# SebastianHafner/greedy_multimodal_learning

Measured on AMD Instinct MI355X. Metric: multi-view images/sec + step ms, ModelNet40 2-view MVCNN+MMTM @1/2/4/8 GPU, higher is better.
Workload: dtype bf16; 1 GPU; C2: 2-view MVCNN(ResNet-18 x2)+MMTM x3, guided gating (training_guided.gin eps 0.01, window 5, unlocked; decided on bf16-trunk gradients: d_BDR within ~6.5e-3 of eps may decide unlike fp32, INTEGRATION.md section 3); params=23773008, global_batch=64, per_gpu_batch=64, image=224, parallelism=dp1, hipgraph=True, device_gate=True

## Files before the change

greedy_multimodal_learning_amd/_lib.py:

```python
import ctypes
import os

import torch

_PKG = os.path.dirname(os.path.abspath(__file__))
LIB_PATH = os.path.join(_PKG, "libgreedymml_hip.so")

GM_F32, GM_BF16 = 0, 1
GM_NCHW, GM_NHWC = 0, 1
ABI_VERSION = 5

c_int, c_float, c_void_p, c_size_t = ctypes.c_int, ctypes.c_float, ctypes.c_void_p, ctypes.c_size_t
c_float_p = ctypes.c_void_p


class SpatialReduce(ctypes.Structure):
    _fields_ = [("x", c_void_p), ("dy", c_void_p), ("C", c_int), ("HW", c_int),
                ("out", c_void_p), ("ld_out", c_int), ("e", c_void_p), ("ld_e", c_int),
                ("scale", c_float)]


class ChannelScale(ctypes.Structure):
    _fields_ = [("x", c_void_p), ("y", c_void_p), ("C", c_int), ("HW", c_int),
                ("s", c_void_p), ("ld_s", c_int), ("a", c_void_p), ("ld_a", c_int),
# ... 104 lines not shown
    "gm_wprep_tiles": (c_int, [c_int, c_int, c_int]),
    "gm_conv_weight_prep_multi_bf16": (c_int, [c_void_p, c_int, c_int, c_void_p]),
})


class ConvDescHW(ctypes.Structure):
    _fields_ = [("N", c_int), ("H", c_int), ("W", c_int), ("C", c_int), ("K", c_int), ("R", c_int), ("S", c_int),
                ("stride_h", c_int), ("stride_w", c_int), ("pad_h", c_int), ("pad_w", c_int)]


EXPORTS.update({
    "gm_conv2d_fwd_hw_bf16": (c_int, [c_void_p, c_void_p, c_void_p, c_void_p, c_void_p]),
    "gm_conv2d_splitk_ws_bytes": (c_size_t, [c_void_p, c_int]),
    "gm_conv2d_fwd_ex_bf16": (c_int, [c_void_p, c_void_p, c_void_p, c_void_p, c_void_p, c_size_t, c_void_p]),
    "gm_conv2d_dgrad_ex_bf16": (c_int, [c_void_p, c_void_p, c_void_p, c_void_p, c_void_p, c_size_t, c_void_p]),
    "gm_conv2d_dgrad_add_bf16": (c_int, [c_void_p, c_void_p, c_void_p, c_void_p, c_void_p, c_void_p, c_size_t,
                                         c_void_p]),
    "gm_conv2d_wgrad_hw_scratch": (c_size_t, [c_void_p]),
    "gm_conv2d_fwd_grouped_bf16": (c_int, [c_void_p, c_int, c_void_p, c_void_p, ctypes.c_longlong, c_void_p,
                                           c_void_p, c_size_t, c_void_p]),
    "gm_conv2d_dgrad_grouped_bf16": (c_int, [c_void_p, c_int, c_void_p, c_void_p, ctypes.c_longlong, c_void_p,
                                             c_void_p, c_void_p, c_size_t, c_void_p]),
    "gm_conv2d_dgrad_grouped_masked_bf16": (c_int, [c_void_p, c_int, c_void_p, c_void_p, ctypes.c_longlong,
                                                    c_void_p, c_void_p, c_void_p, c_void_p, c_size_t, c_void_p]),
    "gm_conv2d_splitk_ws_bytes_grouped": (c_size_t, [c_void_p, c_int, c_int]),
    "gm_conv2d_wgrad_grouped_scratch": (c_size_t, [c_void_p, c_int]),
    "gm_conv2d_wgrad_grouped_bf16": (c_int, [c_void_p, c_int, c_void_p, c_void_p, c_void_p, ctypes.c_longlong,
                                             c_int, c_int, c_void_p, c_size_t, c_void_p]),
    "gm_conv2d_wgrad_hw_bf16": (c_int, [c_void_p, c_void_p, c_void_p, c_void_p, c_int, c_int, c_void_p,
                                        c_size_t, c_void_p]),
    "gm_stem_dw_crop": (c_int, [c_void_p, c_int, c_int, c_int, c_int, c_int, c_int, c_void_p, c_int, c_void_p]),
    "gm_conv2d_wgrad_stem_bn_ok": (c_int, [c_void_p, c_int]),
    "gm_conv2d_wgrad_stem_bn_grouped_bf16": (c_int, [c_void_p, c_int, c_void_p, c_void_p, c_void_p,
                                                     ctypes.c_longlong, c_int, c_void_p, c_size_t, c_void_p]),
})


class StemBnSrc(ctypes.Structure):
    _fields_ = [("y", c_void_p), ("dy_pool", c_void_p), ("idx", c_void_p), ("fcoef", c_void_p),
                ("fcoef_gs", ctypes.c_longlong), ("bcoef", c_void_p), ("bcoef_gs", ctypes.c_longlong)]


class WPrep(ctypes.Structure):
    _fields_ = [("w", c_void_p), ("wb", c_void_p), ("wt", c_void_p), ("K", c_int), ("RS", c_int),
                ("C", c_int), ("Cp", c_int), ("tile_start", c_int), ("pad", c_int)]


class GateState(ctypes.Structure):
    _fields_ = [("curation_mode", c_int), ("caring", c_int), ("curation_step", c_int), ("unlock", c_int),
                ("window", c_int), ("n_curated", c_int), ("pad0", c_int), ("pad1", c_int),
                ("eps", ctypes.c_double), ("M", ctypes.c_double * 4), ("d_bdr", ctypes.c_double)]


GATE_MAX_BRANCHES = 16


class GateStateN(ctypes.Structure):
    _fields_ = [("curation_mode", c_int), ("caring", c_int), ("curation_step", c_int), ("unlock", c_int),
                ("window", c_int), ("n_curated", c_int), ("nb", c_int), ("pad0", c_int),
                ("eps", ctypes.c_double), ("M_bypass", ctypes.c_double * GATE_MAX_BRANCHES),
                ("M_main", ctypes.c_double * GATE_MAX_BRANCHES), ("bdr", ctypes.c_double * GATE_MAX_BRANCHES),
                ("d_bdr", ctypes.c_double)]


class StemPack(ctypes.Structure):
    _fields_ = [("x", c_void_p), ("dtype", c_int), ("N", c_int), ("C0", c_int), ("H", c_int), ("W", c_int),
                ("pad", c_int), ("sn", ctypes.c_longlong), ("sc", ctypes.c_longlong), ("sh", ctypes.c_longlong),
                ("sw", ctypes.c_longlong), ("Hp", c_int), ("Wp", c_int), ("xp", c_void_p), ("w", c_void_p),
                ("K", c_int), ("R", c_int), ("S", c_int), ("wp", c_void_p), ("wk", ctypes.c_longlong),
                ("wc", ctypes.c_longlong), ("wr", ctypes.c_longlong), ("ws", ctypes.c_longlong)]


EXPORTS.update({
    "gm_gate_strong_step": (c_int, [c_void_p, c_void_p, c_void_p]),
    "gm_gate_strong_step_n": (c_int, [c_void_p, c_void_p, c_void_p]),
    "gm_mmtm_channel_scale_gated_n": (c_int, [c_void_p, c_int, c_int, c_int, c_int, c_void_p, c_void_p, c_void_p,
                                              c_void_p]),
    "gm_mmtm_spatial_reduce_gated_n": (c_int, [c_void_p, c_int, c_int, c_int, c_int, c_void_p, c_void_p, c_void_p,
                                               ctypes.c_size_t, c_void_p]),
    "gm_mmtm_select_scale": (c_int, [c_void_p, c_int, c_void_p, c_int, c_void_p, c_void_p, c_int, c_int, c_int,
                                     c_void_p, c_void_p, c_void_p, c_void_p, c_void_p]),
    "gm_mmtm_mask_rows": (c_int, [c_void_p, ctypes.c_longlong, c_void_p, c_void_p]),
    "gm_mmtm_mask_rows2": (c_int, [c_void_p, ctypes.c_longlong, c_void_p, ctypes.c_longlong, c_void_p, c_void_p]),
    "gm_mmtm_channel_scale_gated": (c_int, [c_void_p, c_int, c_int, c_int, c_int, c_void_p, c_void_p, c_void_p,
                                            c_void_p]),
    "gm_mmtm_spatial_reduce_gated": (c_int, [c_void_p, c_int, c_int, c_int, c_int, c_void_p, c_void_p, c_size_t,
                                             c_void_p]),
    "gm_stem_pack_bf16": (c_int, [c_void_p, c_void_p]),
    "gm_stem_pack_grouped_bf16": (c_int, [c_void_p, c_int, c_void_p]),
    "gm_xent_fwd": (c_int, [c_void_p, c_int, c_int, c_int, c_void_p, c_void_p, c_void_p, c_void_p]),
    "gm_xent_bwd": (c_int, [c_void_p, c_void_p, c_int, c_int, c_int, c_void_p, c_void_p, c_void_p, c_void_p]),
})


class BnFwd(ctypes.Structure):
    _fields_ = [("M", ctypes.c_longlong), ("C", c_int), ("relu", c_int), ("x", c_void_p),
                ("residual", c_void_p), ("y", c_void_p), ("gamma", c_void_p), ("beta", c_void_p),
                ("running_mean", c_void_p), ("running_var", c_void_p), ("momentum", c_float),
                ("eps", c_float), ("save_mean", c_void_p), ("save_invstd", c_void_p),
                ("num_batches_tracked", c_void_p), ("coef_out", c_void_p), ("relu_mask", c_void_p)]


class BnBwd(ctypes.Structure):
    _fields_ = [("M", ctypes.c_longlong), ("C", c_int), ("relu", c_int), ("dy", c_void_p),
                ("y", c_void_p), ("x", c_void_p), ("gamma", c_void_p), ("save_mean", c_void_p),
                ("save_invstd", c_void_p), ("dx", c_void_p), ("dres", c_void_p), ("dgamma", c_void_p),
                ("dbeta", c_void_p), ("accumulate", c_int), ("pad", c_int), ("fwd_coef", c_void_p),
                ("relu_mask", c_void_p)]


EXPORTS.update({
    "gm_bn_scratch": (c_size_t, [ctypes.c_longlong, c_int]),
    "gm_bn_fwd_train_bf16": (c_int, [c_void_p, c_void_p, c_size_t, c_void_p]),
    "gm_bn_fwd_stats_bf16": (c_int, [c_void_p, c_void_p, c_size_t, c_void_p]),
    "gm_bn_scratch_grouped": (c_size_t, [ctypes.c_longlong, c_int, c_int]),
    "gm_bn_fwd_train_grouped_bf16": (c_int, [c_void_p, c_int, c_void_p, c_size_t, c_void_p]),
    "gm_bn_bwd_grouped_bf16": (c_int, [c_void_p, c_int, c_void_p, c_size_t, c_void_p]),
    "gm_bn_fwd_stats_grouped_bf16": (c_int, [c_void_p, c_int, c_void_p, c_size_t, c_void_p]),
    "gm_bn_fwd_infer_bf16": (c_int, [c_void_p, c_void_p, c_size_t, c_void_p]),
    "gm_bn_bwd_bf16": (c_int, [c_void_p, c_void_p, c_size_t, c_void_p]),
})


class PoolDesc(ctypes.Structure):
    _fields_ = [("N", c_int), ("H", c_int), ("W", c_int), ("C", c_int), ("k", c_int), ("stride", c_int),
                ("pad", c_int)]


EXPORTS.update({
    "gm_maxpool2d_fwd_bf16": (c_int, [c_void_p, c_void_p, c_void_p, c_void_p, c_void_p]),
    "gm_bn_relu_maxpool2d_fwd_bf16": (c_int, [c_void_p, c_void_p, c_void_p, c_void_p, c_void_p, c_void_p]),
    "gm_bn_relu_maxpool2d_fwd_grouped_bf16": (c_int, [c_void_p, c_int, c_void_p, c_void_p, c_void_p, c_void_p,
                                                      c_void_p, c_void_p]),
    "gm_bn_relu_maxpool2d_bwd_grouped_bf16": (c_int, [c_void_p, c_int, c_void_p, c_void_p, c_void_p, c_void_p,
                                                      c_void_p, c_size_t, c_void_p]),
    "gm_bn_relu_maxpool2d_bwd_stats_grouped_bf16": (c_int, [c_void_p, c_int, c_void_p, c_void_p, c_void_p,
                                                            c_void_p, c_void_p, c_size_t, c_void_p, c_void_p,
                                                            c_void_p]),
    "gm_conv_stem_stats_rows": (c_int, [c_void_p, c_int]),
    "gm_conv2d_fwd_grouped_stats_bf16": (c_int, [c_void_p, c_int, c_void_p, c_void_p, ctypes.c_longlong, c_void_p,
                                                 c_void_p, c_int, c_void_p]),
    "gm_bn_fwd_stats_finalize_grouped": (c_int, [c_void_p, c_int, c_void_p, c_int, c_void_p]),
    "gm_conv2d_fwd_bn_stats_floats": (c_size_t, [c_void_p, c_int]),
    "gm_conv2d_fwd_grouped_bn_stats_bf16": (c_int, [c_void_p, c_int, c_void_p, c_void_p, ctypes.c_longlong, c_void_p,
                                                    c_void_p, c_size_t, c_void_p, c_void_p, c_size_t, c_void_p]),
    "gm_bn_fwd_apply_grouped_bf16": (c_int, [c_void_p, c_int, c_void_p, c_int, c_void_p]),
    "gm_conv2d_dgrad_bn_stats_floats": (c_size_t, [c_void_p, c_int]),
    "gm_conv2d_dgrad_grouped_bn_stats_bf16": (c_int, [c_void_p, c_int, c_void_p, c_void_p, ctypes.c_longlong,
                                                      c_void_p, c_void_p, c_void_p, c_void_p, c_void_p, c_size_t,
                                                      c_void_p, c_void_p, c_size_t, c_void_p]),
    "gm_bn_bwd_stats_coef_offset": (c_size_t, [c_int, c_int, c_int]),
    "gm_bn_bwd_stats_finalize_grouped": (c_int, [c_void_p, c_int, c_void_p, c_int, c_void_p]),
    "gm_bn_bwd_apply_grouped_bf16": (c_int, [c_void_p, c_int, c_void_p, c_int, c_void_p]),
    "gm_maxpool2d_bwd_bf16": (c_int, [c_void_p, c_void_p, c_void_p, c_void_p, c_void_p]),
})


class ConvF32(ctypes.Structure):
    _fields_ = [("mode", c_int), ("d", ConvDesc), ("x", c_void_p), ("w", c_void_p), ("dy", c_void_p),
                ("out", c_void_p), ("addend", c_void_p), ("accumulate", c_int), ("pad0", c_int)]


GM_CONV_FWD, GM_CONV_DGRAD, GM_CONV_WGRAD = 0, 1, 2

EXPORTS.update({
    "gm_conv2d_f32_scratch": (c_size_t, [c_void_p]),
    "gm_conv2d_f32": (c_int, [c_void_p, c_void_p, c_size_t, c_void_p]),
    "gm_conv2d_f32_split_scratch": (c_size_t, [c_void_p, c_int]),
    "gm_conv2d_f32_split": (c_int, [c_void_p, c_int, c_void_p, c_size_t, c_void_p]),
    "gm_conv2d_f32_affine": (c_int, [c_void_p, c_int, c_void_p, c_void_p, c_int, c_void_p, c_size_t, c_void_p]),
    "gm_bn_fwd_train_f32": (c_int, [c_void_p, c_void_p, c_size_t, c_void_p]),
    "gm_bn_fwd_infer_f32": (c_int, [c_void_p, c_void_p, c_size_t, c_void_p]),
    "gm_bn_bwd_f32": (c_int, [c_void_p, c_void_p, c_size_t, c_void_p]),
    "gm_maxpool2d_fwd_f32": (c_int, [c_void_p, c_void_p, c_void_p, c_void_p, c_void_p]),
    "gm_maxpool2d_bwd_f32": (c_int, [c_void_p, c_void_p, c_void_p, c_void_p, c_void_p]),
})

GM_FAULT_BN_SPIN, GM_FAULT_SPLITK_SPIN, GM_FAULT_CHAIN_SPIN = 1, 2, 4

EXPORTS.update({
    "gm_device_faults": (c_int, [ctypes.POINTER(ctypes.c_uint), c_int]),
    "gm_set_spin_limit": (c_int, [ctypes.c_uint]),
    "gm_bn_set_concurrency": (c_int, [c_int]),
    "gm_bn_set_fused_mode": (c_int, [c_int]),
    "gm_set_residency": (c_int, [c_int, c_int, c_int]),
    "gm_get_residency": (c_int, [ctypes.POINTER(c_int), ctypes.POINTER(c_int), ctypes.POINTER(c_int)]),
})


def set_residency(streams=None, sharers=None, reserved_cus=None):
    cur = get_residency()
    new = (cur[0] if streams is None else int(streams), cur[1] if sharers is None else int(sharers),
           cur[2] if reserved_cus is None else int(reserved_cus))
    check(load().gm_set_residency(*new), "gm_set_residency")
    return new


def get_residency():
    a, b, c = c_int(0), c_int(0), c_int(0)
    check(load().gm_get_residency(ctypes.byref(a), ctypes.byref(b), ctypes.byref(c)), "gm_get_residency")
    return a.value, b.value, c.value


_fault_reset_hooks = []


def on_fault_reset(fn):
    _fault_reset_hooks.append(fn)
    return fn


def device_faults(clear=False):
    v = ctypes.c_uint(0)
    check(load().gm_device_faults(ctypes.byref(v), int(clear)), "gm_device_faults")
    return v.value


def check_device_faults(clear=True):
    v = device_faults(clear)
    if v:
        for hook in _fault_reset_hooks:
            hook()
        what = [n for b, n in ((GM_FAULT_BN_SPIN, "fused BatchNorm coefficient hand-off"),
                               (GM_FAULT_SPLITK_SPIN, "split-K convolution turnstile"),
                               (GM_FAULT_CHAIN_SPIN, "chained GEMM hand-off")) if v & b]
        raise GreedyMMLError(f"device fault 0x{v:x}: {', '.join(what) or 'unknown'} timed out "
                             "(grid not co-resident?); the affected outputs are NaN")


class ViewsNorm(ctypes.Structure):
    _fields_ = [("x", c_void_p), ("flip", c_void_p), ("B", c_int), ("V", c_int), ("H", c_int), ("W", c_int),
                ("C", c_int), ("mean", c_float * 4), ("std", c_float * 4), ("out", c_void_p), ("dtype", c_int),
                ("layout", c_int)]


EXPORTS.update({
    "gm_views_normalize": (c_int, [c_void_p, c_void_p]),
})

EXPORTS.update({
    "gm_conv_set_halo": (c_int, [c_int]),
    "gm_conv_set_h9": (c_int, [c_int]),
    "gm_conv_set_wgrad_staging": (c_int, [c_int]),
    "gm_conv_set_splitk": (c_int, [c_int]),
    "gm_conv_set_wgrad_loop": (c_int, [c_int]),
    "gm_conv_set_1x1_gemm": (c_int, [c_int]),
    "gm_conv_set_rw": (c_int, [c_int]),
    "gm_conv_set_stem": (c_int, [c_int]),
    "gm_conv_set_wgrad_stem": (c_int, [c_int]),
})


class BnCoefEntry(ctypes.Structure):
    _fields_ = [("gamma", c_void_p), ("beta", c_void_p), ("running_mean", c_void_p), ("running_var", c_void_p),
                ("coef", c_void_p), ("C", c_int), ("eps", c_float)]


EXPORTS.update({
    "gm_bn_infer_coef": (c_int, [c_void_p, c_int, c_int, c_void_p]),
    "gm_conv2d_fwd_affine_ok": (c_int, [c_void_p, c_int]),
    "gm_conv2d_fwd_grouped_affine_bf16": (c_int, [c_void_p, c_int, c_void_p, c_void_p, ctypes.c_longlong, c_void_p,
                                                  c_void_p, ctypes.c_longlong, c_void_p, c_int, c_void_p, c_size_t,
                                                  c_void_p]),
    "gm_eval_metrics": (c_int, [c_void_p, c_int, c_int, c_int, c_void_p, c_void_p, c_void_p]),
})
```

greedy_multimodal_learning_amd/csrc/batchnorm.hip:

```cpp
#include <cstdlib>
#include <initializer_list>
#include <type_traits>

#include "gm_common.h"

namespace gm {
namespace {

constexpr int kT = 256;
constexpr int kMaxC = 2048;
constexpr size_t kHdr = 256;
constexpr int kMaxRC = 512;
constexpr int kRedF = 4096;

struct Plan {
    int SW, tpr_log, rpp;
    int nslice, nrc;
    long long rpb;
    size_t off_coef, off_p1, bytes;
};

inline int ilog2(int v) {
    int l = 0;
    while ((1 << l) < v) ++l;
// ... 98 lines not shown
    const float* gamma;
    const float* beta;
    float* rmean;
    float* rvar;
    float momentum, eps;
    float* save_mean;
    float* save_invstd;
    float* dgamma;
    float* dbeta;
    unsigned* counter;
    long long* nbt;
    float* coef;
    float* part;
    float* coef_out;
    const float* fcoef;
    unsigned* gen;
    const uint4* res;
    uint4* yout;
    uint4* dres_out;
    uint8_t* mask_out;
    const uint8_t* ymask;
    unsigned spin_limit;
    int redundant;
    unsigned long long scr_stride;
    unsigned hdr_words;
    BnGroup grp[kMaxBnG];
};

__device__ __forceinline__ ReduceArgs group_args(const ReduceArgs& a0) {
    ReduceArgs a = a0;
    const int g = blockIdx.z;
    const BnGroup& q = a0.grp[g];
    a.x = q.x; a.dy = q.dy; a.y = q.y;
    a.gamma = q.gamma; a.beta = q.beta; a.rmean = q.rmean; a.rvar = q.rvar;
    a.save_mean = q.save_mean; a.save_invstd = q.save_invstd;
    a.dgamma = q.dgamma; a.dbeta = q.dbeta; a.nbt = q.nbt;
    a.coef_out = q.coef_out; a.fcoef = q.fcoef;
    a.res = q.res; a.yout = q.yout; a.dres_out = q.dres_out;
    a.mask_out = q.mask_out; a.ymask = q.ymask;
    const unsigned long long off = (unsigned long long)g * a0.scr_stride;
    a.counter = a0.counter + g * a0.hdr_words;
    a.coef = reinterpret_cast<float*>(reinterpret_cast<char*>(a0.coef) + off);
    a.part = reinterpret_cast<float*>(reinterpret_cast<char*>(a0.part) + off);
    if (a0.gen) a.gen = a0.gen + g * a0.hdr_words;
    return a;
}

__device__ unsigned g_bn_fault = 0;

__device__ __forceinline__ bool wait_generation(const unsigned* gen, unsigned g0, unsigned limit, float* flag) {
    if (threadIdx.x == 0) {
        unsigned it = 0;
        bool ok = true;
        while (__hip_atomic_load(gen, __ATOMIC_RELAXED, __HIP_MEMORY_SCOPE_AGENT) == g0) {
            if (++it >= limit) {
                ok = false;
                break;
            }
            __builtin_amdgcn_s_sleep(2);
        }
        if (!ok) atomicOr(&g_bn_fault, GM_FAULT_BN_SPIN);
        *flag = ok ? 1.f : 0.f;
    }
    __syncthreads();
    return *flag != 0.f;
}

enum { FWD = 0, BWD = 1, BWD_RELU = 2, BWD_RELUX = 3 };

template <int MODE, typename E>
__device__ __forceinline__ void accum(const ReduceArgs& a, long long v, const float* mu, float* s1, float* s2,
                                      const float* fsc, const float* fsh) {
    float xf[8];
    V8<E>::ld(a.x, v, xf);
    if (MODE == FWD) {
#pragma unroll
        for (int j = 0; j < 8; ++j) {
            s1[j] += xf[j];
            s2[j] = fmaf(xf[j], xf[j], s2[j]);
        }
    } else {
        float d[8];
        V8<E>::ld(a.dy, v, d);
        if (MODE == BWD_RELU) {
            float yf[8];
            V8<E>::ld(a.y, v, yf);
#pragma unroll
            for (int j = 0; j < 8; ++j) d[j] = yf[j] > 0.f ? d[j] : 0.f;
        }
        if (MODE == BWD_RELUX) {
#pragma unroll
            for (int j = 0; j < 8; ++j) d[j] = fmaf(xf[j], fsc[j], fsh[j]) > 0.f ? d[j] : 0.f;
        }
#pragma unroll
        for (int j = 0; j < 8; ++j) {
            s1[j] += d[j];
            s2[j] = fmaf(d[j], xf[j] - mu[j], s2[j]);
        }
    }
}

template <int MODE>
__device__ __forceinline__ void accum_vals(uint4 ux, uint4 ud, uint4 uy, const float* mu, float* s1, float* s2,
                                          const float* fsc = nullptr, const float* fsh = nullptr) {
    float xf[8];
    unpack8(ux, xf);
    if (MODE == FWD) {
#pragma unroll
        for (int j = 0; j < 8; ++j) {
            s1[j] += xf[j];
            s2[j] = fmaf(xf[j], xf[j], s2[j]);
        }
    } else {
        float d[8];
        unpack8(ud, d);
        if (MODE == BWD_RELU) {
            float yf[8];
            unpack8(uy, yf);
#pragma unroll
            for (int j = 0; j < 8; ++j) d[j] = yf[j] > 0.f ? d[j] : 0.f;
        }
        if (MODE == BWD_RELUX) {
#pragma unroll
            for (int j = 0; j < 8; ++j) d[j] = fmaf(xf[j], fsc[j], fsh[j]) > 0.f ? d[j] : 0.f;
        }
#pragma unroll
        for (int j = 0; j < 8; ++j) {
            s1[j] += d[j];
            s2[j] = fmaf(d[j], xf[j] - mu[j], s2[j]);
        }
    }
}

struct FinOps {
    float g, b, rm, rv;
};

template <int MODE>
__device__ __forceinline__ FinOps fin_load(const ReduceArgs& a, int c) {
    FinOps f;
    f.g = a.gamma[c];
    if (MODE == FWD) {
        f.b = a.beta[c];
        f.rm = a.rmean ? a.rmean[c] : 0.f;
        f.rv = a.rmean ? a.rvar[c] : 0.f;
    } else {
        f.b = 0.f;
        f.rm = a.save_mean[c];
        f.rv = a.save_invstd[c];
    }
    return f;
}

template <int MODE, bool SC1 = false, bool CENTER = false>
__device__ __forceinline__ void finalize(const ReduceArgs& a, int c, double S1, double S2, double invM,
                                         const FinOps& f) {
    const int C = a.C;
    const double g = (double)f.g;
    if (MODE == FWD) {
        const double mean = S1 * invM;
        double var = S2 * invM - mean * mean;
        if (var < 0.0) var = 0.0;
        const double invstd = 1.0 / sqrt(var + (double)a.eps);
        const double sc = g * invstd;
        a.coef[c] = (float)sc;
        a.coef[C + c] = (float)((double)f.b - mean * sc);
        if (SC1) {
            st_sc1(&a.coef[c], a.coef[c]);
            st_sc1(&a.coef[C + c], a.coef[C + c]);
        }
        if (a.coef_out) {
            a.coef_out[c] = a.coef[c];
            a.coef_out[C + c] = a.coef[C + c];
        }
        a.save_mean[c] = (float)mean;
        a.save_invstd[c] = (float)invstd;
        if (a.rmean) {
            const double m = (double)a.momentum;
            const double unb = a.M > 1 ? var * (double)a.M / (double)(a.M - 1) : var;
            a.rmean[c] = (float)((1.0 - m) * (double)f.rm + m * mean);
            a.rvar[c] = (float)((1.0 - m) * (double)f.rv + m * unb);
        }
    } else {
        const double mean = (double)f.rm;
        const double is = (double)f.rv;
        const double ca = g * is;
        const double cb = -g * is * is * is * S2 * invM;
        a.coef[c] = (float)ca;
        a.coef[C + c] = (float)cb;
        if (CENTER) {
            a.coef[2 * C + c] = (float)(-ca * S1 * invM);
            a.coef[3 * C + c] = (float)mean;
        } else {
            a.coef[2 * C + c] = (float)(-ca * S1 * invM - cb * mean);
        }
        if (SC1) {
            st_sc1(&a.coef[c], a.coef[c]);
            st_sc1(&a.coef[C + c], a.coef[C + c]);
            st_sc1(&a.coef[2 * C + c], a.coef[2 * C + c]);
        }
        const float dg = (float)(S2 * is), db = (float)S1;
        if (a.accumulate) {
            a.dgamma[c] += dg;
            a.dbeta[c] += db;
        } else {
            a.dgamma[c] = dg;
            a.dbeta[c] = db;
        }
    }
}


__device__ __forceinline__ bool ticket(unsigned* ctr, unsigned n, float* flag) {
    asm volatile("s_waitcnt vmcnt(0)" ::: "memory");
    __syncthreads();
    if (threadIdx.x == 0) {
        const unsigned tk = __hip_atomic_fetch_add(ctr, 1u, __ATOMIC_RELAXED, __HIP_MEMORY_SCOPE_AGENT);
        const bool last = tk == n - 1;
        if (last) __hip_atomic_store(ctr, 0u, __ATOMIC_RELAXED, __HIP_MEMORY_SCOPE_AGENT);
        *flag = last ? 1.f : 0.f;
    }
    __syncthreads();
    return *flag != 0.f;
}

template <int MODE, bool SC1 = false>
__device__ __forceinline__ void combine_finalize(const ReduceArgs& a, int cs, float* red, const FinOps& fo);

template <int MODE, typename E>
__global__ __launch_bounds__(kT) void k_bn_reduce(ReduceArgs a0) {
    const ReduceArgs a = group_args(a0);
    __shared__ float red[kRedF + 4];
    const int t = threadIdx.x;
    const int C = a.C, SW = a.SW;
    const int rc = blockIdx.x, cs = blockIdx.y;
    const int tpr = 1 << a.tpr_log;
    const int cg = t & (tpr - 1);
    const int r0 = t >> a.tpr_log;
    const int rpp = kT >> a.tpr_log;
    const long long vpr = C >> 3;
    const int c0 = cs * SW + cg * 8;

    float fsc[8], fsh[8];
    if (MODE == BWD_RELUX) {
#pragma unroll
        for (int j = 0; j < 8; ++j) {
            fsc[j] = a.fcoef[c0 + j];
            fsh[j] = a.fcoef[C + c0 + j];
        }
    }
    float mu[8];
    if (MODE != FWD) {
#pragma unroll
        for (int j = 0; j < 8; ++j) mu[j] = a.save_mean[c0 + j];
    }
    float s1[8], s2[8];
#pragma unroll
    for (int j = 0; j < 8; ++j) s1[j] = s2[j] = 0.f;

    const long long rbeg = (long long)rc * a.rpb;
    long long rend = rbeg + a.rpb;
    if (rend > a.M) rend = a.M;
    long long r = rbeg + r0;
    const long long cv = c0 >> 3;
    const long long st = (long long)rpp * vpr;
    for (; r + 7 * rpp < rend; r += 8 * rpp) {
        const long long v = r * vpr + cv;
#pragma unroll
        for (int u = 0; u < 8; ++u) accum<MODE, E>(a, v + u * st, mu, s1, s2, fsc, fsh);
    }
    if (MODE == FWD && std::is_same<E, uint16_t>::value && r < rend) {
        const uint4* X = static_cast<const uint4*>(a.x);
        uint4 vx[8];
        const uint4 z = make_uint4(0u, 0u, 0u, 0u);
#pragma unroll
        for (int u = 0; u < 8; ++u) vx[u] = X[(r + u * rpp < rend ? r + u * rpp : r) * vpr + cv];
#pragma unroll
        for (int u = 0; u < 8; ++u) accum_vals<MODE>(r + u * rpp < rend ? vx[u] : z, z, z, mu, s1, s2);
    } else {
        for (; r < rend; r += rpp) accum<MODE, E>(a, r * vpr + cv, mu, s1, s2, fsc, fsh);
    }

    const int S2w = 2 * SW;
#pragma unroll
    for (int j = 0; j < 8; ++j) {
        red[r0 * S2w + (cg * 8 + j) * 2] = s1[j];
        red[r0 * S2w + (cg * 8 + j) * 2 + 1] = s2[j];
    }
    __syncthreads();
    float* p1 = a.part + ((size_t)cs * a.nrc + rc) * S2w;
    if (t < S2w) {
        float acc = 0.f;
        for (int i = 0; i < rpp; ++i) acc += red[i * S2w + t];
        st_sc1(&p1[t], acc);
    }
    FinOps fo{};
    if (t < SW) fo = fin_load<MODE>(a, cs * SW + t);
    if (!ticket(a.counter + cs, (unsigned)a.nrc, &red[kRedF])) return;
    combine_finalize<MODE>(a, cs, red, fo);
}

template <int MODE, bool SC1>
__device__ __forceinline__ void combine_finalize(const ReduceArgs& a, int cs, float* red, const FinOps& fo) {
    const int t = threadIdx.x;
    const int SW = a.SW, S2w = 2 * SW;
    if (MODE == FWD && a.nbt && cs == 0 && t == 0) *a.nbt += 1;
    const int L = S2w >> 2, G = kT / L;
    const int lv = t % L, g = t / L;
    const auto rq = rsrc_of(a.part + (size_t)cs * a.nrc * S2w);
    double d0 = 0.0, d1 = 0.0, d2 = 0.0, d3 = 0.0;
    for (int i0 = g; i0 < a.nrc; i0 += 8 * G) {
        float4 v[8];
#pragma unroll
        for (int u = 0; u < 8; ++u) {
            const int i = i0 + u * G;
            v[u] = i < a.nrc ? ld_sc1_f32x4(rq, (unsigned)(i * S2w + 4 * lv) * 4u) : make_float4(0.f, 0.f, 0.f, 0.f);
        }
#pragma unroll
        for (int u = 0; u < 8; ++u) {
            d0 += (double)v[u].x; d1 += (double)v[u].y; d2 += (double)v[u].z; d3 += (double)v[u].w;
        }
    }
    __syncthreads();
    double* rd = reinterpret_cast<double*>(red);
    rd[g * S2w + 4 * lv + 0] = d0;
    rd[g * S2w + 4 * lv + 1] = d1;
    rd[g * S2w + 4 * lv + 2] = d2;
    rd[g * S2w + 4 * lv + 3] = d3;
    __syncthreads();
    if (t < SW) {
        double S1 = 0.0, S2 = 0.0;
        for (int i = 0; i < G; ++i) {
            S1 += rd[i * S2w + 2 * t];
            S2 += rd[i * S2w + 2 * t + 1];
        }
        finalize<MODE, SC1>(a, cs * SW + t, S1, S2, 1.0 / (double)a.M, fo);
    }
}

struct StemPoolGeo {
    int Ng, H, W, P, Q;
    long long items;
    long long ipb;
    const uint2* idx;
    const uint4* gp;
    const uint4* xs;
};

typedef unsigned u32x4v_t __attribute__((ext_vector_type(4)));
__device__ __forceinline__ uint4 ld_nt16(const uint4* p) {
    const u32x4v_t v = __builtin_nontemporal_load(reinterpret_cast<const u32x4v_t*>(p));
    return make_uint4(v.x, v.y, v.z, v.w);
}
__device__ __forceinline__ void st_nt16(uint4* p, uint4 v) {
    const u32x4v_t w = {v.x, v.y, v.z, v.w};
    __builtin_nontemporal_store(w, reinterpret_cast<u32x4v_t*>(p));
}

template <bool APPLY>
__global__ __launch_bounds__(kT) void k_stem_pool_bn_bwd(ReduceArgs a0, StemPoolGeo pg) {
    const ReduceArgs a = group_args(a0);
    __shared__ float red[kRedF + 4];
// ... 24 lines not shown
    for (int j = 0; j < 8; ++j) s1[j] = s2[j] = 0.f;
    struct Item {
        uint2 iv[4];
        uint4 gq[4], xv[4];
        int n, k, l, cg;
        unsigned okw;
    };
    const unsigned QC8 = (unsigned)pg.Q * C8, WC8 = (unsigned)pg.W * C8;
    auto load = [&](long long i64, Item& it) {
        const unsigned i = (unsigned)i64;
        const unsigned ob = i / (unsigned)C8;
        it.cg = (int)(i - ob * (unsigned)C8);
        const unsigned r1 = ob / (unsigned)pg.Q;
        it.l = (int)(ob - r1 * (unsigned)pg.Q);
        const unsigned nn = r1 / (unsigned)pg.P;
        it.k = (int)(r1 - nn * (unsigned)pg.P);
        it.n = (int)nn;
        const int k = it.k, l = it.l;
        const unsigned o0 = i;
        it.okw = 0u;
#pragma unroll
        for (int u = 0; u < 4; ++u) {
            const int wr = u >> 1, wc = u & 1;
            const bool ok = k + wr < pg.P && l + wc < pg.Q;
            const unsigned o = ok ? o0 + (unsigned)wr * QC8 + (unsigned)wc * (unsigned)C8 : o0;
            it.iv[u] = IDX[o];
            it.gq[u] = GP[o];
            it.okw |= ok ? (1u << u) : 0u;
        }
        const unsigned x0 = ((nn * (unsigned)pg.H + 2u * (unsigned)k) * (unsigned)pg.W + 2u * (unsigned)l) * C8 + it.cg;
#pragma unroll
        for (int q = 0; q < 4; ++q) {
            const int dh = q >> 1, dw = q & 1;
            const bool in = 2 * k + dh < pg.H && 2 * l + dw < pg.W;
            it.xv[q] = ld_nt16(&X[in ? x0 + (unsigned)dh * WC8 + (unsigned)dw * (unsigned)C8 : x0]);
        }
    };
    auto compute = [&](const Item& it) {
        const int n = it.n, k = it.k, l = it.l, cg = it.cg;
        float gv[4][8];
#pragma unroll
        for (int u = 0; u < 4; ++u) unpack8(it.gq[u], gv[u]);
        uint2 ivm[4];
#pragma unroll
        for (int u = 0; u < 4; ++u) ivm[u] = ((it.okw >> u) & 1u) ? it.iv[u] : make_uint2(~0u, ~0u);
#pragma unroll
        for (int q = 0; q < 4; ++q) {
            const int dh = q >> 1, dw = q & 1;
            const int h = 2 * k + dh, w = 2 * l + dw;
            if (h >= pg.H || w >= pg.W) continue;
            float d[8];
#pragma unroll
            for (int j = 0; j < 8; ++j) d[j] = 0.f;
#pragma unroll
            for (int u = 0; u < 4; ++u) {
                const int wr = u >> 1, wc = u & 1;
                if (wr > dh || wc > dw) continue;
                const uint32_t pos = (uint32_t)((dh - 2 * wr + 1) * 3 + (dw - 2 * wc + 1));
#pragma unroll
                for (int j = 0; j < 8; ++j) {
                    const uint32_t b = ((j < 4 ? ivm[u].x : ivm[u].y) >> (8 * (j & 3))) & 0xffu;
                    if (b == pos) d[j] += gv[u][j];
                }
            }
            float xf[8];
            unpack8(it.xv[q], xf);
#pragma unroll
            for (int j = 0; j < 8; ++j) {
                const float dr = __uint_as_float((uint32_t)Elem<uint16_t>::f2bf(d[j]) << 16);
                d[j] = fmaf(xf[j], fsc[j], fsh[j]) > 0.f ? dr : 0.f;
            }
            if (APPLY) {
                float o[8];
#pragma unroll
                for (int j = 0; j < 8; ++j) o[j] = fmaf(ca[j], d[j], fmaf(cb[j], xf[j], cc[j]));
                st_nt16(&reinterpret_cast<uint4*>(a.yout)[(((long long)n * pg.H + h) * pg.W + w) * C8 + cg], pack8(o));
            } else {
#pragma unroll
                for (int j = 0; j < 8; ++j) {
                    s1[j] += d[j];
                    s2[j] = fmaf(d[j], xf[j] - mu[j], s2[j]);
                }
            }
        }
    };
    auto item = [&](long long i) {
        Item it;
        load(i, it);
        compute(it);
    };
    if (APPLY) {
        const long long stride = (long long)gridDim.x * kT;
        long long i = (long long)blockIdx.x * kT + t;
        for (; i + stride < pg.items; i += 2 * stride) {
            Item u, v;
            load(i, u);
            load(i + stride, v);
            compute(u);
            compute(v);
        }
        if (i < pg.items) item(i);
        return;
    }
    const int rc = blockIdx.x;
    const long long i0 = (long long)rc * pg.ipb;
    const long long i1 = i0 + pg.ipb < pg.items ? i0 + pg.ipb : pg.items;
    if (pg.xs) {
        const uint4* __restrict__ XS = pg.xs + goff;
        for (long long i = i0 + t; i < i1; i += 4 * kT) {
            uint4 gq[4], xq[4];
#pragma unroll
            for (int u = 0; u < 4; ++u) {
                const long long iu = i + u * kT < i1 ? i + u * kT : i;
                gq[u] = GP[iu];
                xq[u] = XS[iu];
            }
#pragma unroll
            for (int u = 0; u < 4; ++u) {
                if (i + u * kT >= i1) break;
                float gv[8], xf[8];
                unpack8(gq[u], gv);
                unpack8(xq[u], xf);
#pragma unroll
                for (int j = 0; j < 8; ++j) {
                    const float d = fmaf(xf[j], fsc[j], fsh[j]) > 0.f ? gv[j] : 0.f;
                    s1[j] += d;
                    s2[j] = fmaf(d, xf[j] - mu[j], s2[j]);
                }
            }
        }
    } else {
        for (long long i = i0 + t; i < i1; i += kT) item(i);
    }
    const int S2w = 2 * C, r0 = t / C8, rpp = kT / C8;
#pragma unroll
    for (int j = 0; j < 8; ++j) {
        red[r0 * S2w + (cg0 * 8 + j) * 2] = s1[j];
        red[r0 * S2w + (cg0 * 8 + j) * 2 + 1] = s2[j];
    }
    __syncthreads();
    float* p1 = a.part + (size_t)rc * S2w;
    if (t < S2w) {
        float acc = 0.f;
        for (int i = 0; i < rpp; ++i) acc += red[i * S2w + t];
        st_sc1(&p1[t], acc);
    }
    FinOps fo{};
    if (t < C) fo = fin_load<BWD_RELUX>(a, t);
    if (!ticket(a.counter, (unsigned)a.nrc, &red[kRedF])) return;
    combine_finalize<BWD_RELUX>(a, 0, red, fo);
}

constexpr int kFinT = 1024;
__global__ __launch_bounds__(kFinT) void k_bn_stats_finalize(ReduceArgs a0) {
    const ReduceArgs a = group_args(a0);
    __shared__ double rd[kFinT / 32][128];
    const int t = threadIdx.x, cs = blockIdx.y;
    const int lv = t & 31, rg = t >> 5;
    FinOps fo;
    {
        const int c = cs * 64 + (t & 63);
        const float* rm = a.rmean ? a.rmean : a.gamma;
        const float* rv = a.rmean ? a.rvar : a.gamma;
        fo.g = a.gamma[c];
        fo.b = a.beta[c];
        fo.rm = rm[c];
        fo.rv = rv[c];
    }
    const float4* rows = reinterpret_cast<const float4*>(a.part + (size_t)cs * a.nrc * 128);
    double d0 = 0.0, d1 = 0.0, d2 = 0.0, d3 = 0.0;
    for (int i0 = rg; i0 < a.nrc; i0 += 8 * 32) {
        float4 v[8];
#pragma unroll
        for (int u = 0; u < 8; ++u) v[u] = rows[(size_t)min(i0 + u * 32, a.nrc - 1) * 32 + lv];
#pragma unroll
        for (int u = 0; u < 8; ++u) {
            if (i0 + u * 32 >= a.nrc) v[u] = make_float4(0.f, 0.f, 0.f, 0.f);
            d0 += (double)v[u].x; d1 += (double)v[u].y; d2 += (double)v[u].z; d3 += (double)v[u].w;
        }
    }
    rd[rg][4 * lv] = d0; rd[rg][4 * lv + 1] = d1; rd[rg][4 * lv + 2] = d2; rd[rg][4 * lv + 3] = d3;
    __syncthreads();
    if (t < 64) {
        double S1 = 0.0, S2 = 0.0;
        for (int i = 0; i < kFinT / 32; ++i) {
            S1 += rd[i][2 * t];
            S2 += rd[i][2 * t + 1];
        }
        finalize<FWD>(a, cs * 64 + t, S1, S2, 1.0 / (double)a.M, fo);
        if (a.nbt && cs == 0 && t == 0) *a.nbt += 1;
    }
}

__global__ __launch_bounds__(kFinT) void k_bn_bwd_stats_finalize(ReduceArgs a0, float* coef0, long long cstride) {
    ReduceArgs a = group_args(a0);
    a.coef = coef0 + blockIdx.z * cstride;
    __shared__ double rd[kFinT / 32][128];
    const int t = threadIdx.x, cs = blockIdx.y;
    const int lv = t & 31, rg = t >> 5;
    const FinOps fo = fin_load<BWD>(a, cs * 64 + (t & 63));
    const float4* rows = reinterpret_cast<const float4*>(a.part + (size_t)cs * a.nrc * 128);
    double d0 = 0.0, d1 = 0.0, d2 = 0.0, d3 = 0.0;
    for (int i0 = rg; i0 < a.nrc; i0 += 8 * 32) {
        float4 v[8];
#pragma unroll
        for (int u = 0; u < 8; ++u) v[u] = rows[(size_t)min(i0 + u * 32, a.nrc - 1) * 32 + lv];
#pragma unroll
        for (int u = 0; u < 8; ++u) {
            if (i0 + u * 32 >= a.nrc) v[u] = make_float4(0.f, 0.f, 0.f, 0.f);
            d0 += (double)v[u].x; d1 += (double)v[u].y; d2 += (double)v[u].z; d3 += (double)v[u].w;
        }
    }
    rd[rg][4 * lv] = d0; rd[rg][4 * lv + 1] = d1; rd[rg][4 * lv + 2] = d2; rd[rg][4 * lv + 3] = d3;
    __syncthreads();
    if (t < 64) {
        double S1 = 0.0, S2 = 0.0;
        for (int i = 0; i < kFinT / 32; ++i) {
            S1 += rd[i][2 * t];
            S2 += rd[i][2 * t + 1];
        }
        finalize<BWD>(a, cs * 64 + t, S1, S2, 1.0 / (double)a.M, fo);
    }
}

__device__ __forceinline__ bool arrive(unsigned* ctr, unsigned n, float* flag) {
    asm volatile("s_waitcnt vmcnt(0)" ::: "memory");
    __syncthreads();
    if (threadIdx.x == 0) {
        const unsigned tk = __hip_atomic_fetch_add(ctr, 1u, __ATOMIC_RELAXED, __HIP_MEMORY_SCOPE_AGENT);
        *flag = tk == n - 1 ? 1.f : 0.f;
    }
    __syncthreads();
    return *flag != 0.f;
}

__device__ __forceinline__ bool wait_count(unsigned* ctr, unsigned n, unsigned limit, float* flag) {
    if (threadIdx.x == 0) {
        unsigned it = 0;
        bool ok = true;
        while (__hip_atomic_load(ctr, __ATOMIC_RELAXED, __HIP_MEMORY_SCOPE_AGENT) < n) {
            if (++it >= limit) {
                ok = false;
                break;
            }
            __builtin_amdgcn_s_sleep(1);
        }
        if (!ok) atomicOr(&g_bn_fault, GM_FAULT_BN_SPIN);
        *flag = ok ? 1.f : 0.f;
    }
    __syncthreads();
    return *flag != 0.f;
}

__device__ __forceinline__ void depart(unsigned* ctr, unsigned n) {
    if (threadIdx.x == 0) {
        const unsigned tk = __hip_atomic_fetch_add(ctr, 1u, __ATOMIC_RELAXED, __HIP_MEMORY_SCOPE_AGENT);
        if (tk == 2 * n - 1) __hip_atomic_store(ctr, 0u, __ATOMIC_RELAXED, __HIP_MEMORY_SCOPE_AGENT);
    }
}

template <int MODE>
__device__ __forceinline__ void combine_coefs(const ReduceArgs& a, int cs, float* red, const FinOps& fo, bool last,
                                              float* cf) {
    const int t = threadIdx.x;
    const int SW = a.SW, S2w = 2 * SW;
    const int L = S2w >> 2, G = kT / L;
    const int lv = t % L, g = t / L;
    const auto rq = rsrc_of(a.part + (size_t)cs * a.nrc * S2w);
    double d0 = 0.0, d1 = 0.0, d2 = 0.0, d3 = 0.0;
    for (int i0 = g; i0 < a.nrc; i0 += 8 * G) {
        float4 v[8];
#pragma unroll
        for (int u = 0; u < 8; ++u) {
            const int i = i0 + u * G;
            v[u] = i < a.nrc ? ld_sc1_f32x4(rq, (unsigned)(i * S2w + 4 * lv) * 4u) : make_float4(0.f, 0.f, 0.f, 0.f);
        }
#pragma unroll
        for (int u = 0; u < 8; ++u) {
            d0 += (double)v[u].x; d1 += (double)v[u].y; d2 += (double)v[u].z; d3 += (double)v[u].w;
        }
    }
    __syncthreads();
    double* rd = reinterpret_cast<double*>(red);
    rd[g * S2w + 4 * lv + 0] = d0;
    rd[g * S2w + 4 * lv + 1] = d1;
    rd[g * S2w + 4 * lv + 2] = d2;
    rd[g * S2w + 4 * lv + 3] = d3;
    __syncthreads();
    if (t < SW) {
        double S1 = 0.0, S2 = 0.0;
        for (int i = 0; i < G; ++i) {
            S1 += rd[i * S2w + 2 * t];
            S2 += rd[i * S2w + 2 * t + 1];
        }
        const double invM = 1.0 / (double)a.M;
        const int c = cs * SW + t;
        if (last) {
            if (MODE == FWD && a.nbt && cs == 0 && t == 0) *a.nbt += 1;
            finalize<MODE, false>(a, c, S1, S2, invM, fo);
        }
        const double gg = (double)fo.g;
        if (MODE == FWD) {
            const double mean = S1 * invM;
            double var = S2 * invM - mean * mean;
            if (var < 0.0) var = 0.0;
            const double invstd = 1.0 / sqrt(var + (double)a.eps);
            const double sc = gg * invstd;
            cf[t] = (float)sc;
            cf[SW + t] = (float)((double)fo.b - mean * sc);
        } else {
            const double mean = (double)fo.rm, is = (double)fo.rv;
            const double ca = gg * is, cb = -gg * is * is * is * S2 * invM;
            cf[t] = (float)ca;
            cf[SW + t] = (float)cb;
            cf[2 * SW + t] = (float)(-ca * S1 * invM - cb * mean);
        }
    }
    __syncthreads();
}

template <int MODE>
__global__ __launch_bounds__(kT) void k_bn_reduce_f64(ReduceArgs a0) {
    const ReduceArgs a = group_args(a0);
    __shared__ double red[kRedF];
    __shared__ float flag;
    const int t = threadIdx.x;
    const int C = a.C, SW = a.SW;
    const int rc = blockIdx.x, cs = blockIdx.y;
    const int tpr = 1 << a.tpr_log;
    const int cg = t & (tpr - 1);
    const int r0 = t >> a.tpr_log;
    const int rpp = kT >> a.tpr_log;
    const long long vpr = C >> 3;
    const int c0 = cs * SW + cg * 8;
    const float* X = static_cast<const float*>(a.x);
    const float* DY = static_cast<const float*>(a.dy);
    const float* Y = static_cast<const float*>(a.y);
    double fsc[8], fsh[8], mu[8], s1[8], s2[8];
#pragma unroll
    for (int j = 0; j < 8; ++j) {
        fsc[j] = MODE == BWD_RELUX ? (double)a.fcoef[c0 + j] : 0.0;
        fsh[j] = MODE == BWD_RELUX ? (double)a.fcoef[C + c0 + j] : 0.0;
        mu[j] = MODE != FWD ? (double)a.save_mean[c0 + j] : 0.0;
        s1[j] = s2[j] = 0.0;
    }
    const long long rbeg = (long long)rc * a.rpb;
    long long rend = rbeg + a.rpb;
    if (rend > a.M) rend = a.M;
    for (long long r = rbeg + r0; r < rend; r += rpp) {
        const long long e = r * C + c0;
        float xf[8], d[8];
        V8<float>::ld(X + e, 0, xf);
        if (MODE != FWD) V8<float>::ld(DY + e, 0, d);
        if (MODE == BWD_RELU) {
            float yf[8];
            V8<float>::ld(Y + e, 0, yf);
#pragma unroll
            for (int j = 0; j < 8; ++j) d[j] = yf[j] > 0.f ? d[j] : 0.f;
        }
#pragma unroll
        for (int j = 0; j < 8; ++j) {
            if (MODE == BWD_RELUX) d[j] = fmaf(xf[j], (float)fsc[j], (float)fsh[j]) > 0.f ? d[j] : 0.f;
            if (MODE == FWD) {
                s1[j] += (double)xf[j];
                s2[j] = fma((double)xf[j], (double)xf[j], s2[j]);
            } else {
                s1[j] += (double)d[j];
                s2[j] = fma((double)d[j], (double)xf[j] - mu[j], s2[j]);
            }
        }
    }
    const int S2w = 2 * SW;
#pragma unroll
    for (int j = 0; j < 8; ++j) {
// ... 217 lines not shown
            unsigned wm[US];
#pragma unroll
            for (int u = 0; u < US; ++u) {
                const long long i = r * vpr + cv + u * st;
                wx[u] = X[i];
                wd[u] = DY[i];
                if (MODE == BWD_RELU && YM) wm[u] = a.ymask[i];
                else if (MODE == BWD_RELU) wy[u] = Y[i];
            }
#pragma unroll
            for (int u = 0; u < US; ++u) {
                pin(wx[u]);
                pin(wd[u]);
                if (MODE == BWD_RELU && YM) pin(wm[u]);
                else if (MODE == BWD_RELU) pin(wy[u]);
            }
#pragma unroll
            for (int u = 0; u < US; ++u)
                accum_vals<MODE>(wx[u], wd[u], MODE == BWD_RELU ? (YM ? mask_vals(wm[u]) : wy[u]) : z, mu, s1, s2, fsc,
                                 fsh);
        }
        for (; r < rend; r += rpp) {
            const long long i = r * vpr + cv;
            accum_vals<MODE>(X[i], DY[i], MODE == BWD_RELU ? ldy(i) : z, mu, s1, s2, fsc, fsh);
        }
    }

    const int S2w = 2 * SW;
#pragma unroll
    for (int j = 0; j < 8; ++j) {
        red[r0 * S2w + (cg * 8 + j) * 2] = s1[j];
        red[r0 * S2w + (cg * 8 + j) * 2 + 1] = s2[j];
    }
    __syncthreads();
    float* p1 = a.part + ((size_t)cs * a.nrc + rc) * S2w;
    if (t < S2w) {
        float acc = 0.f;
        for (int i = 0; i < rpp; ++i) acc += red[i * S2w + t];
        st_sc1(&p1[t], acc);
    }
    FinOps fo{};
    if (t < SW) fo = fin_load<MODE>(a, cs * SW + t);
    bool fresh = true;
    float ca[8], cb[8], cc[8];
    if (a.redundant) {
        __shared__ float cf[3 * 64];
        const bool last = arrive(a.counter + cs, (unsigned)a.nrc, &red[kRedF]);
        fresh = wait_count(a.counter + cs, (unsigned)a.nrc, a.spin_limit, &red[kRedF + 1]);
        combine_coefs<MODE>(a, cs, red, fo, last, cf);
        depart(a.counter + cs, (unsigned)a.nrc);
#pragma unroll
        for (int j = 0; j < 8; ++j) {
            ca[j] = cf[cg * 8 + j];
            cb[j] = cf[SW + cg * 8 + j];
            cc[j] = cf[2 * SW + cg * 8 + j];
        }
    } else {
        if (ticket(a.counter + cs, (unsigned)a.nrc, &red[kRedF])) {
            combine_finalize<MODE, true>(a, cs, red, fo);
            asm volatile("s_waitcnt vmcnt(0)" ::: "memory");
            __syncthreads();
            if (t == 0) __hip_atomic_store(gen, g0 + 1u, __ATOMIC_RELAXED, __HIP_MEMORY_SCOPE_AGENT);
        } else {
            fresh = wait_generation(gen, g0, a.spin_limit, &red[kRedF + 1]);
        }
        const auto rq = rsrc_of(a.coef);
        auto ld8 = [&](int off, float* o) {
            const float4 p = ld_sc1_f32x4(rq, (unsigned)(off + c0) * 4u), q = ld_sc1_f32x4(rq, (unsigned)(off + c0 + 4) * 4u);
            o[0] = p.x; o[1] = p.y; o[2] = p.z; o[3] = p.w; o[4] = q.x; o[5] = q.y; o[6] = q.z; o[7] = q.w;
        };
        ld8(0, ca);
        ld8(C, cb);
        ld8(2 * C, cc);
    }
    if (!fresh) {
#pragma unroll
        for (int j = 0; j < 8; ++j) ca[j] = cb[j] = cc[j] = __builtin_nanf("");
    }
    auto out = [&](uint4 ux, uint4 ud, uint4 uy, long long i) {
        float d[8], xf[8];
        unpack8(ud, d);
        unpack8(ux, xf);
        if (MODE == BWD_RELU) {
            float yf[8];
            unpack8(uy, yf);
#pragma unroll
            for (int j = 0; j < 8; ++j) d[j] = yf[j] > 0.f ? d[j] : 0.f;
        }
        if (MODE == BWD_RELUX) {
#pragma unroll
            for (int j = 0; j < 8; ++j) d[j] = fmaf(xf[j], fsc[j], fsh[j]) > 0.f ? d[j] : 0.f;
        }
        if (DRES) a.dres_out[i] = pack8(d);
        float o[8];
#pragma unroll
        for (int j = 0; j < 8; ++j)
            o[j] = fmaf(ca[j], d[j], fmaf(cb[j], xf[j], cc[j]));
        a.yout[i] = pack8(o);
    };
    if (NR > 0) {
#pragma unroll
        for (int u = 0; u < NV; ++u) {
            const long long r = rbeg + r0 + (long long)u * rpp;
            if (r < rend) out(vx[u], vd[u], MODE == BWD_RELU ? vy[u < NY ? u : 0] : z, r * vpr + cv);
        }
    } else {
        long long r = rbeg + r0;
        const long long st = (long long)rpp * vpr;
        for (; r + (US - 1) * rpp < rend; r += US * rpp) {
            uint4 wx[US], wd[US], wy[US];
            unsigned wm[US];
#pragma unroll
            for (int u = 0; u < US; ++u) {
                const long long i = r * vpr + cv + u * st;
                wx[u] = X[i];
                wd[u] = DY[i];
                if (MODE == BWD_RELU && YM) wm[u] = a.ymask[i];
                else if (MODE == BWD_RELU) wy[u] = Y[i];
            }
#pragma unroll
            for (int u = 0; u < US; ++u) {
                pin(wx[u]);
                pin(wd[u]);
                if (MODE == BWD_RELU && YM) pin(wm[u]);
                else if (MODE == BWD_RELU) pin(wy[u]);
            }
#pragma unroll
            for (int u = 0; u < US; ++u)
                out(wx[u], wd[u], MODE == BWD_RELU ? (YM ? mask_vals(wm[u]) : wy[u]) : z, r * vpr + cv + u * st);
        }
        for (; r < rend; r += rpp) {
            const long long i = r * vpr + cv;
            out(X[i], DY[i], MODE == BWD_RELU ? ldy(i) : z, i);
        }
    }
}

struct ApplyArgs {
    long long nvec;
    int tpr_log;
    int relu;
    const void* x;
    const void* res;
    const void* dy;
    void* out;
    void* out2;
    const float* coef;
    int C;
    const float* fcoef;
    long long gvec;
    long long cgs;
    long long fcgs;
    uint8_t* mask_out;
};

__device__ __forceinline__ void load_coef(const float* p, int cg, float* c) {
    const float4 a = reinterpret_cast<const float4*>(p)[cg * 2];
    const float4 b = reinterpret_cast<const float4*>(p)[cg * 2 + 1];
    c[0] = a.x; c[1] = a.y; c[2] = a.z; c[3] = a.w; c[4] = b.x; c[5] = b.y; c[6] = b.z; c[7] = b.w;
}

template <bool RES, bool RELU, typename E>
__global__ __launch_bounds__(kT) void k_bn_apply(ApplyArgs a) {
    const long long stride = (long long)gridDim.x * kT;
    long long v = (long long)blockIdx.x * kT + threadIdx.x;
    const int cg = (int)(v & ((1 << a.tpr_log) - 1));
    const long long go = blockIdx.y * a.gvec;
    const float* coef = a.coef + blockIdx.y * a.cgs;
    float sc[8], sh[8];
    load_coef(coef, cg, sc);
    load_coef(coef + a.C, cg, sh);
    auto fin = [&](long long i, float* f, const float* r) {
#pragma unroll
        for (int j = 0; j < 8; ++j) {
            float z = fmaf(f[j], sc[j], sh[j]);
            if (RES) z += r[j];
            f[j] = RELU ? relu_nan(z) : z;
        }
        V8<E>::st(a.out, i, f);
        if (RES && RELU && std::is_same<E, uint16_t>::value && a.mask_out) a.mask_out[i] = (uint8_t)mask_byte(pack8(f));
    };
    auto one = [&](long long i) {
        i += go;
        float f[8];
        V8<E>::ld(a.x, i, f);
        float r[8];
        if (RES) V8<E>::ld(a.res, i, r);
        fin(i, f, r);
    };
    if constexpr (std::is_same<E, uint16_t>::value) {
        typedef unsigned u32x4 __attribute__((ext_vector_type(4)));
        constexpr int U = 4;
        const u32x4* XX = static_cast<const u32x4*>(a.x) + go;
        const u32x4* RR = static_cast<const u32x4*>(a.res) + go;
        for (; v + (U - 1) * stride < a.nvec; v += U * stride) {
            u32x4 rx[U], rr[U];
#pragma unroll
            for (int u = 0; u < U; ++u) {
                rx[u] = XX[v + u * stride];
                if (RES) rr[u] = RR[v + u * stride];
            }
#pragma unroll
            for (int u = 0; u < U; ++u) {
                asm volatile("" : "+v"(rx[u]));
                if (RES) asm volatile("" : "+v"(rr[u]));
            }
#pragma unroll
            for (int u = 0; u < U; ++u) {
                float f[8], r[8];
                unpack8(make_uint4(rx[u].x, rx[u].y, rx[u].z, rx[u].w), f);
                if (RES) unpack8(make_uint4(rr[u].x, rr[u].y, rr[u].z, rr[u].w), r);
                fin(go + v + u * stride, f, r);
            }
        }
        for (; v < a.nvec; v += stride) one(v);
        return;
    }
    for (; v + stride < a.nvec; v += 2 * stride) {
        one(v);
        one(v + stride);
    }
    if (v < a.nvec) one(v);
}

template <bool RELU, bool DRES, bool MASKX, typename E>
__global__ __launch_bounds__(kT) void k_bn_apply_bwd(ApplyArgs a) {
    constexpr bool CENTER = std::is_same<E, float>::value;
    const long long stride = (long long)gridDim.x * kT;
    long long v = (long long)blockIdx.x * kT + threadIdx.x;
    const int cg = (int)(v & ((1 << a.tpr_log) - 1));
    const long long go = blockIdx.y * a.gvec;
    const float* coef = a.coef + blockIdx.y * a.cgs;
    float ca[8], cb[8], cc[8], fs[8], fh[8], mu[8];
    load_coef(coef, cg, ca);
    load_coef(coef + a.C, cg, cb);
    load_coef(coef + 2 * a.C, cg, cc);
    if (CENTER) load_coef(coef + 3 * a.C, cg, mu);
    if (MASKX) {
        load_coef(a.fcoef + blockIdx.y * a.fcgs, cg, fs);
        load_coef(a.fcoef + blockIdx.y * a.fcgs + a.C, cg, fh);
    }
    constexpr bool YR = RELU && !MASKX;
    auto ld = [&](long long i, float* d, float* xf, float* yf) {
        V8<E>::ld(a.dy, go + i, d);
        V8<E>::ld(a.x, go + i, xf);
        if (YR) V8<E>::ld(a.res, go + i, yf);
    };
    auto out = [&](long long i, float* d, const float* xf, const float* yf) {
        if (RELU && MASKX) {
#pragma unroll
            for (int j = 0; j < 8; ++j) d[j] = fmaf(xf[j], fs[j], fh[j]) > 0.f ? d[j] : 0.f;
        } else if (RELU) {
#pragma unroll
            for (int j = 0; j < 8; ++j) d[j] = yf[j] > 0.f ? d[j] : 0.f;
        }
        if (DRES) V8<E>::st(a.out2, go + i, d);
        float o[8];
#pragma unroll
        for (int j = 0; j < 8; ++j)
            o[j] = CENTER ? fmaf(ca[j], d[j], fmaf(cb[j], xf[j] - mu[j], cc[j])) : fmaf(ca[j], d[j], fmaf(cb[j], xf[j], cc[j]));
        V8<E>::st(a.out, go + i, o);
    };
    constexpr int U = 4;
    if constexpr (std::is_same<E, uint16_t>::value) {
        typedef unsigned u32x4 __attribute__((ext_vector_type(4)));
        const u32x4* DY = static_cast<const u32x4*>(a.dy) + go;
        const u32x4* XX = static_cast<const u32x4*>(a.x) + go;
        const u32x4* YY = static_cast<const u32x4*>(a.res) + go;
        auto u4 = [](u32x4 w) { return make_uint4(w.x, w.y, w.z, w.w); };
        for (; v + (U - 1) * stride < a.nvec; v += U * stride) {
            u32x4 rd[U], rx[U], ry[U];
#pragma unroll
            for (int u = 0; u < U; ++u) {
                rd[u] = DY[v + u * stride];
                rx[u] = XX[v + u * stride];
                if (YR) ry[u] = YY[v + u * stride];
            }
#pragma unroll
            for (int u = 0; u < U; ++u) {
                asm volatile("" : "+v"(rd[u]), "+v"(rx[u]));
                if (YR) asm volatile("" : "+v"(ry[u]));
            }
#pragma unroll
            for (int u = 0; u < U; ++u) {
                float d[8], xf[8], yf[8];
                unpack8(u4(rd[u]), d);
                unpack8(u4(rx[u]), xf);
                if (YR) unpack8(u4(ry[u]), yf);
                out(v + u * stride, d, xf, yf);
            }
        }
    } else {
        for (; v + (U - 1) * stride < a.nvec; v += U * stride) {
            float d[U][8], xf[U][8], yf[U][YR ? 8 : 1];
#pragma unroll
            for (int u = 0; u < U; ++u) ld(v + u * stride, d[u], xf[u], yf[u]);
#pragma unroll
            for (int u = 0; u < U; ++u) out(v + u * stride, d[u], xf[u], yf[u]);
        }
    }
    for (; v < a.nvec; v += stride) {
        float d[8], xf[8], yf[YR ? 8 : 1];
        ld(v, d, xf, yf);
        out(v, d, xf, yf);
    }
}

__global__ void k_bn_infer_coef(int C, const float* gamma, const float* beta, const float* rm, const float* rv,
                                float eps, float* coef) {
    const int c = blockIdx.x * blockDim.x + threadIdx.x;
    if (c >= C) return;
    const double is = 1.0 / sqrt((double)rv[c] + (double)eps);
    const double sc = (double)gamma[c] * is;
    coef[c] = (float)sc;
    coef[C + c] = (float)((double)beta[c] - (double)rm[c] * sc);
}

__global__ void k_bn_infer_coef_table(const gm_bn_coef_entry* tab) {
    const gm_bn_coef_entry e = tab[blockIdx.y];
    const int c = blockIdx.x * blockDim.x + threadIdx.x;
    const int C = e.C;
    if (c >= C) return;
    const double is = 1.0 / sqrt((double)e.running_var[c] + (double)e.eps);
    const double sc = (double)e.gamma[c] * is;
    e.coef[c] = (float)sc;
// ... 397 lines not shown
    ReduceArgs a{};
    fill_fwd(a, ps, G, grouped, pl, static_cast<char*>(scratch));
    hipLaunchKernelGGL((k_bn_reduce<FWD, uint16_t>), dim3(pl.nrc, pl.nslice, G), dim3(kT), 0, as_stream(stream), a);
    return check_launch("k_bn_reduce<fwd>");
}

}

namespace gm {
unsigned bn_faults_read(bool clear) {
    unsigned v = 0;
    if (hipMemcpyFromSymbol(&v, HIP_SYMBOL(g_bn_fault), sizeof(v), 0, hipMemcpyDeviceToHost) != hipSuccess) return ~0u;
    if (clear && v) {
        const unsigned z = 0;
        (void)hipMemcpyToSymbol(HIP_SYMBOL(g_bn_fault), &z, sizeof(z), 0, hipMemcpyHostToDevice);
    }
    return v;
}
}

extern "C" int gm_bn_set_concurrency(int n) {
    GM_REQUIRE(n >= 1 && n <= 1024, "gm_bn_set_concurrency: n must be in [1, 1024] (got %d)", n);
    gm::g_concurrency = n;
    return GM_OK;
}

extern "C" int gm_bn_set_fused_mode(int mode) {
    GM_REQUIRE(mode >= 0 && mode <= 2, "gm_bn_set_fused_mode: mode must be 0, 1 or 2 (got %d)", mode);
    gm::g_fused_env = mode;
    return GM_OK;
}

extern "C" int gm_bn_fwd_stats_bf16(const gm_bn_fwd* p, void* scratch, size_t bytes, void* stream) {
    return bn_fwd_stats(p, 1, false, scratch, bytes, stream, "gm_bn_fwd_stats_bf16");
}

extern "C" size_t gm_bn_scratch_grouped(long long M, int C, int G) {
    if (M <= 0 || C < 8 || C > kMaxC || G < 1 || G > kMaxBnG) return 0;
    return grouped_bytes(M, C, G);
}

extern "C" int gm_bn_fwd_train_grouped_bf16(const gm_bn_fwd* ps, int G, void* scratch, size_t bytes, void* stream) {
    return bn_fwd_train<uint16_t>(ps, G, true, scratch, bytes, stream, "gm_bn_fwd_train_grouped_bf16");
}
extern "C" int gm_bn_bwd_grouped_bf16(const gm_bn_bwd* ps, int G, void* scratch, size_t bytes, void* stream) {
    return bn_bwd<uint16_t>(ps, G, true, scratch, bytes, stream, "gm_bn_bwd_grouped_bf16");
}
extern "C" int gm_bn_fwd_stats_grouped_bf16(const gm_bn_fwd* ps, int G, void* scratch, size_t bytes, void* stream) {
    return bn_fwd_stats(ps, G, true, scratch, bytes, stream, "gm_bn_fwd_stats_grouped_bf16");
}

extern "C" int gm_bn_fwd_train_bf16(const gm_bn_fwd* p, void* scratch, size_t bytes, void* stream) {
    return bn_fwd_train<uint16_t>(p, 1, false, scratch, bytes, stream, "gm_bn_fwd_train_bf16");
}
extern "C" int gm_bn_fwd_infer_bf16(const gm_bn_fwd* p, void* scratch, size_t bytes, void* stream) {
    return bn_fwd_infer<uint16_t>(p, scratch, bytes, stream, "gm_bn_fwd_infer_bf16");
}
extern "C" int gm_bn_bwd_bf16(const gm_bn_bwd* p, void* scratch, size_t bytes, void* stream) {
    return bn_bwd<uint16_t>(p, 1, false, scratch, bytes, stream, "gm_bn_bwd_bf16");
}
extern "C" int gm_bn_fwd_train_f32(const gm_bn_fwd* p, void* scratch, size_t bytes, void* stream) {
    return bn_fwd_train<float>(p, 1, false, scratch, bytes, stream, "gm_bn_fwd_train_f32");
}
extern "C" int gm_bn_infer_coef(const gm_bn_coef_entry* table, int n, int max_c, void* stream) {
    const char* fn = "gm_bn_infer_coef";
    GM_REQUIRE(table, "%s: null table", fn);
    GM_REQUIRE(n >= 1 && n <= 65535, "%s: n must be 1..65535 (got %d)", fn, n);
    GM_REQUIRE(max_c >= 1, "%s: max_c must be >= 1 (got %d)", fn, max_c);
    hipLaunchKernelGGL(k_bn_infer_coef_table, dim3((max_c + 255) / 256, n), dim3(256), 0, as_stream(stream), table);
    return check_launch("k_bn_infer_coef_table");
}

extern "C" int gm_bn_fwd_infer_f32(const gm_bn_fwd* p, void* scratch, size_t bytes, void* stream) {
    return bn_fwd_infer<float>(p, scratch, bytes, stream, "gm_bn_fwd_infer_f32");
}
extern "C" int gm_bn_bwd_f32(const gm_bn_bwd* p, void* scratch, size_t bytes, void* stream) {
    return bn_bwd<float>(p, 1, false, scratch, bytes, stream, "gm_bn_bwd_f32");
}

static int stem_pool_bwd(const gm_pool_desc* d, int G, const void* dy_pool, const void* idx, const void* xsel,
                         const gm_bn_bwd* ps, void* scratch, size_t bytes, bool apply, const float** bcoef,
                         long long* bcoef_gs, void* stream, const char* fn) {
    GM_REQUIRE(d && dy_pool && idx && ps && G >= 1 && G <= kMaxBnG, "%s: bad arguments", fn);
    GM_REQUIRE(d->k == 3 && d->stride == 2 && d->pad == 1 && d->C == 64 && d->N >= 1 && d->H >= 2 && d->W >= 2,
               "%s: the stem's pool only (k 3, stride 2, pad 1, C 64)", fn);
    const int P = (d->H + 2 - 3) / 2 + 1, Q = (d->W + 2 - 3) / 2 + 1;
    GM_REQUIRE((d->H + 1) / 2 == P && (d->W + 1) / 2 == Q, "%s: pool geometry", fn);
    for (int g = 0; g < G; ++g) {
        const gm_bn_bwd& p = ps[g];
        GM_REQUIRE(p.M == (long long)d->N * d->H * d->W && p.C == d->C && p.relu && p.fwd_coef && !p.y && !p.dres &&
                       p.x && (p.dx || !apply) && p.gamma && p.save_mean && p.save_invstd && p.dgamma && p.dbeta &&
                       p.accumulate == ps[0].accumulate,
                   "%s: group %d: BN backward must be M = N*H*W, C, relu with fwd_coef, no y / dres", fn, g);
    }
    int rc;
    if ((rc = check_scratch(ps[0].M, ps[0].C, G, true, scratch, bytes, fn))) return rc;
    const Plan pl = make_plan(ps[0].M, ps[0].C);
    ReduceArgs a{};
    a.M = ps[0].M; a.C = ps[0].C; a.relu = 1; a.SW = ps[0].C; a.tpr_log = 3;
    a.accumulate = ps[0].accumulate;
    set_scratch(a, pl, static_cast<char*>(scratch), true);
    for (int g = 0; g < G; ++g) {
        BnGroup& q = a.grp[g];
        q.x = ps[g].x;
        q.gamma = ps[g].gamma;
        q.save_mean = const_cast<float*>(ps[g].save_mean);
        q.save_invstd = const_cast<float*>(ps[g].save_invstd);
        q.dgamma = ps[g].dgamma; q.dbeta = ps[g].dbeta;
        q.fcoef = ps[g].fwd_coef;
        q.yout = static_cast<uint4*>(ps[g].dx);
    }
    StemPoolGeo pg;
    pg.Ng = d->N; pg.H = d->H; pg.W = d->W; pg.P = P; pg.Q = Q;
    pg.items = (long long)d->N * P * Q * (d->C / 8);
    GM_REQUIRE((long long)d->N * d->H * d->W * (d->C / 8) < (1ll << 31), "%s: a group's map exceeds 2^31 vectors", fn);
    int nrc = pl.nrc < kMaxRC ? pl.nrc : kMaxRC;
    pg.ipb = (pg.items + nrc - 1) / nrc;
    pg.ipb = (pg.ipb + kT - 1) / kT * kT;
    nrc = (int)((pg.items + pg.ipb - 1) / pg.ipb);
    a.nrc = nrc;
    pg.idx = static_cast<const uint2*>(idx);
    pg.gp = static_cast<const uint4*>(dy_pool);
    pg.xs = static_cast<const uint4*>(xsel);
    hipStream_t st = as_stream(stream);
    hipLaunchKernelGGL((k_stem_pool_bn_bwd<false>), dim3(nrc, 1, G), dim3(kT), 0, st, a, pg);
    if ((rc = check_launch("k_stem_pool_bn_bwd<reduce>"))) return rc;
    if (!apply) {
        *bcoef = a.coef;
        *bcoef_gs = (long long)(a.scr_stride / sizeof(float));
        return GM_OK;
    }
    long long grid = (pg.items + kT - 1) / kT;
    if (grid > 4096) grid = 4096;
    hipLaunchKernelGGL((k_stem_pool_bn_bwd<true>), dim3((unsigned)grid, 1, G), dim3(kT), 0, st, a, pg);
    return check_launch("k_stem_pool_bn_bwd<apply>");
}

extern "C" int gm_bn_relu_maxpool2d_bwd_grouped_bf16(const gm_pool_desc* d, int G, const void* dy_pool,
                                                     const void* idx, const void* xsel, const gm_bn_bwd* ps,
                                                     void* scratch, size_t bytes, void* stream) {
    return stem_pool_bwd(d, G, dy_pool, idx, xsel, ps, scratch, bytes, true, nullptr, nullptr, stream,
                         "gm_bn_relu_maxpool2d_bwd_grouped_bf16");
}

extern "C" int gm_bn_relu_maxpool2d_bwd_stats_grouped_bf16(const gm_pool_desc* d, int G, const void* dy_pool,
                                                           const void* idx, const void* xsel, const gm_bn_bwd* ps,
                                                           void* scratch, size_t bytes, const float** bcoef,
                                                           long long* bcoef_gs, void* stream) {
    const char* fn = "gm_bn_relu_maxpool2d_bwd_stats_grouped_bf16";
    GM_REQUIRE(bcoef && bcoef_gs, "%s: null coefficient outputs", fn);
    return stem_pool_bwd(d, G, dy_pool, idx, xsel, ps, scratch, bytes, false, bcoef, bcoef_gs, stream, fn);
}

extern "C" int gm_bn_fwd_stats_finalize_grouped(const gm_bn_fwd* ps, int G, float* stats, int rows, void* stream) {
    const char* fn = "gm_bn_fwd_stats_finalize_grouped";
    int rc = check_groups_fwd(ps, G, fn);
    if (rc) return rc;
    const int C = ps[0].C;
    GM_REQUIRE(stats && rows >= 1 && C >= 64 && C % 64 == 0 && ps[0].M >= 1, "%s: C a multiple of 64, rows >= 1",
               fn);
    ReduceArgs a{};
    a.M = ps[0].M; a.C = C; a.SW = 64; a.tpr_log = 3; a.nrc = rows;
    a.momentum = ps[0].momentum; a.eps = ps[0].eps;
    a.part = stats;
    a.coef = stats + (size_t)rows * 2 * C;
    a.scr_stride = (unsigned long long)(rows + 1) * 2 * C * sizeof(float);
    a.hdr_words = 0;
    for (int g = 0; g < G; ++g) {
        BnGroup& q = a.grp[g];
        q.x = ps[g].x;
        q.gamma = ps[g].gamma; q.beta = ps[g].beta;
        q.rmean = ps[g].running_mean; q.rvar = ps[g].running_var;
        q.save_mean = ps[g].save_mean; q.save_invstd = ps[g].save_invstd;
        q.nbt = ps[g].num_batches_tracked;
        q.coef_out = ps[g].coef_out;
    }
    hipLaunchKernelGGL(k_bn_stats_finalize, dim3(1, C / 64, G), dim3(kFinT), 0, as_stream(stream), a);
    return check_launch("k_bn_stats_finalize");
}

extern "C" int gm_bn_fwd_apply_grouped_bf16(const gm_bn_fwd* ps, int G, const float* stats, int rows, void* stream) {
    const char* fn = "gm_bn_fwd_apply_grouped_bf16";
    int rc = check_groups_fwd(ps, G, fn);
    if (rc) return rc;
    const gm_bn_fwd* p = ps;
    const int C = p->C;
    GM_REQUIRE(stats && rows >= 1 && C >= 64 && C % 64 == 0 && p->y, "%s: C a multiple of 64, rows >= 1, y", fn);
    const long long gs = p->M * C;
    bool strided = true;
    for (int g = 1; g < G; ++g) {
        const uint16_t* x0 = static_cast<const uint16_t*>(p->x);
        strided = strided && ps[g].x == x0 + g * gs &&
                  ps[g].y == static_cast<uint16_t*>(p->y) + g * gs &&
                  (!p->residual || ps[g].residual == static_cast<const uint16_t*>(p->residual) + g * gs) &&
                  (!p->relu_mask || ps[g].relu_mask == static_cast<uint8_t*>(p->relu_mask) + g * gs / 8);
    }
    const long long cgs = (long long)(rows + 1) * 2 * C;
    hipStream_t st = as_stream(stream);
    const int ng = strided ? 1 : G;
    for (int gi = 0; gi < ng; ++gi) {
        ApplyArgs b{};
        b.nvec = p->M * (C / 8); b.tpr_log = ilog2(C / 8); b.C = C; b.relu = p->relu;
        b.x = ps[gi].x; b.res = ps[gi].residual; b.out = ps[gi].y;
        b.mask_out = static_cast<uint8_t*>(ps[gi].relu_mask);
        b.coef = stats + gi * cgs + (size_t)rows * 2 * C;
        b.gvec = strided ? gs / 8 : 0;
        b.cgs = strided ? cgs : 0;
        const dim3 g(apply_grid(b.nvec, C), strided ? G : 1);
        if (p->residual) {
            if (p->relu) hipLaunchKernelGGL((k_bn_apply<true, true, uint16_t>), g, dim3(kT), 0, st, b);
            else hipLaunchKernelGGL((k_bn_apply<true, false, uint16_t>), g, dim3(kT), 0, st, b);
        } else {
            if (p->relu) hipLaunchKernelGGL((k_bn_apply<false, true, uint16_t>), g, dim3(kT), 0, st, b);
            else hipLaunchKernelGGL((k_bn_apply<false, false, uint16_t>), g, dim3(kT), 0, st, b);
        }
        if ((rc = check_launch("k_bn_apply"))) return rc;
    }
    return GM_OK;
}

extern "C" size_t gm_bn_bwd_stats_coef_offset(int C, int G, int rows) {
    return (size_t)G * 2 * C * (size_t)(rows + 1);
}

static int check_bwd_from_stats(const gm_bn_bwd* ps, int G, const float* stats, int rows, const char* fn) {
    int rc = check_groups_bwd(ps, G, fn);
    if (rc) return rc;
    const int C = ps[0].C;
    GM_REQUIRE(stats && rows >= 1 && C >= 64 && C % 64 == 0 && ps[0].M >= 1, "%s: C a multiple of 64, rows >= 1",
               fn);
    GM_REQUIRE(!ps[0].dres && (!ps[0].relu || ps[0].fwd_coef),
               "%s: relu needs fwd_coef (mask from x); no residual gradient", fn);
    return GM_OK;
}

extern "C" int gm_bn_bwd_stats_finalize_grouped(const gm_bn_bwd* ps, int G, float* stats, int rows, void* stream) {
    const char* fn = "gm_bn_bwd_stats_finalize_grouped";
    int rc = check_bwd_from_stats(ps, G, stats, rows, fn);
    if (rc) return rc;
    const int C = ps[0].C;
    ReduceArgs a{};
    a.M = ps[0].M; a.C = C; a.SW = 64; a.tpr_log = 3; a.nrc = rows;
    a.accumulate = ps[0].accumulate;
    a.part = stats;
    a.coef = stats;
    a.scr_stride = (unsigned long long)(rows + 1) * 2 * C * sizeof(float);
    a.hdr_words = 0;
    for (int g = 0; g < G; ++g) {
        BnGroup& q = a.grp[g];
        q.x = ps[g].x; q.dy = ps[g].dy;
        q.gamma = ps[g].gamma;
        q.save_mean = const_cast<float*>(ps[g].save_mean);
        q.save_invstd = const_cast<float*>(ps[g].save_invstd);
        q.dgamma = ps[g].dgamma; q.dbeta = ps[g].dbeta;
    }
    float* coef0 = stats + gm_bn_bwd_stats_coef_offset(C, G, rows);
    hipLaunchKernelGGL(k_bn_bwd_stats_finalize, dim3(1, C / 64, G), dim3(kFinT), 0, as_stream(stream), a, coef0,
                       (long long)4 * C);
    return check_launch("k_bn_bwd_stats_finalize");
}

extern "C" int gm_bn_bwd_apply_grouped_bf16(const gm_bn_bwd* ps, int G, const float* stats, int rows, void* stream) {
    const char* fn = "gm_bn_bwd_apply_grouped_bf16";
    int rc = check_bwd_from_stats(ps, G, stats, rows, fn);
    if (rc) return rc;
    const gm_bn_bwd* p = ps;
    const int C = p->C;
    GM_REQUIRE(p->dx && p->dy && p->x, "%s: null argument (dx, dy, x)", fn);
    const long long gs = p->M * C;
    bool strided = true;
    for (int g = 1; g < G; ++g)
        strided = strided && ps[g].x == static_cast<const uint16_t*>(p->x) + g * gs &&
                  ps[g].dy == static_cast<const uint16_t*>(p->dy) + g * gs &&
                  ps[g].dx == static_cast<uint16_t*>(p->dx) + g * gs &&
                  (!p->relu || ps[g].fwd_coef == p->fwd_coef + (size_t)g * 2 * C);
    const float* coef0 = stats + gm_bn_bwd_stats_coef_offset(C, G, rows);
    hipStream_t st = as_stream(stream);
    const int ng = strided ? 1 : G;
    for (int gi = 0; gi < ng; ++gi) {
        ApplyArgs b{};
        b.nvec = p->M * (C / 8); b.tpr_log = ilog2(C / 8); b.C = C; b.relu = p->relu;
        b.x = ps[gi].x; b.dy = ps[gi].dy; b.out = ps[gi].dx;
        b.coef = coef0 + (size_t)gi * 4 * C;
        b.fcoef = ps[gi].fwd_coef;
        b.gvec = strided ? gs / 8 : 0;
        b.cgs = strided ? 4 * C : 0;
        b.fcgs = strided ? 2 * C : 0;
        const dim3 g(apply_grid(b.nvec, C), strided ? G : 1);
        if (p->relu) hipLaunchKernelGGL((k_bn_apply_bwd<true, false, true, uint16_t>), g, dim3(kT), 0, st, b);
        else hipLaunchKernelGGL((k_bn_apply_bwd<false, false, false, uint16_t>), g, dim3(kT), 0, st, b);
        if ((rc = check_launch("k_bn_apply_bwd"))) return rc;
    }
    return GM_OK;
}
```

greedy_multimodal_learning_amd/vtrunk.py:

```python
import contextlib
import ctypes
import os

import torch

from .streams import zeroed_scratch
from . import _lib as L
from .bn import MASK_FROM_X
from .conv import CL, _cpad, _desc, _desc_hw, _like_param, _prepped, _splitk_ws, _stem_geom, stem_pack, \
    stem_pack_grouped
from .gradsink import GradJoin, MaskedAddend, sink_done, sink_pending, sink_target

BF = torch.bfloat16
ENABLED = os.environ.get("GM_VTRUNK", "1") != "0"


FUSED_STEM_BWD = True
STEM_XSEL = True
FUSED_STEM_WGRAD = True
FUSED_STEM_STATS = True
EPI_BN_STATS = True
BN_RELU_MASK = True
DS_DZ_LINK = True
IDT_MASKED_ADDEND = True
EPI_BN_BWD_STATS = True
_GM_E_UNSUP = -3


def _nhwc(t):
    return t if t.is_contiguous(memory_format=CL) else t.contiguous(memory_format=CL)


def _stride(ts, elem_bytes):
    if len(ts) < 2:
        return 0
    d = ts[1].data_ptr() - ts[0].data_ptr()
    if d == 0 or d % elem_bytes:
        return None
    for a, b in zip(ts[1:], ts[2:]):
        if b.data_ptr() - a.data_ptr() != d:
            return None
    return d // elem_bytes


def _splitk_g(device, d, G, dgrad):
    need = L.load().gm_conv2d_splitk_ws_bytes_grouped(ctypes.byref(d), G, int(dgrad))
    if need == 0:
        return 0, 0
    buf = zeroed_scratch(_splitk_ws, device, need, lambda old: (need + (1 << 20) - 1) >> 20 << 20)
    return buf.data_ptr(), buf.numel()


_bn_scratch = {}


def _bn_scratch_g(device, M, C, G):
    need = L.load().gm_bn_scratch_grouped(M, C, G)
    return zeroed_scratch(_bn_scratch, device, need,
                          lambda old: max(need, 1 << 20) if old is None else max(need, 2 * old.numel()))


@L.on_fault_reset
def _reset_bn_scratch():
    for buf in _bn_scratch.values():
        buf.zero_()
    torch.cuda.synchronize()



WGRAD_STREAM = True
_WGRAD_SIDE = 64
WGRAD_BATCH = 8
_PENDING = []


def flush_wgrads():
    if not _PENDING:
        return
    items = list(_PENDING)
    _PENDING.clear()
    dev = items[0][3]
    side = _wgrad_stream(dev)
    if side is not None:
        side.wait_stream(torch.cuda.current_stream(dev))
    with torch.cuda.stream(side) if side is not None else contextlib.nullcontext():
        for launch, _, keep, _ in items:
            if side is not None:
                for t in keep:
                    t.record_stream(side)
            launch()
    for _, weights, _, _ in items:
        for w in weights:
            sink_done(w)


def drop_pending_wgrads():
    n = len(_PENDING)
    _PENDING.clear()
    return n


def _defer_wgrad(launch, weights, keep, dev):
    for w in weights:
        sink_pending(w)
    if not _PENDING:
        torch.autograd.Variable._execution_engine.queue_callback(flush_wgrads)
    _PENDING.append((launch, weights, keep, dev))
    if len(_PENDING) >= WGRAD_BATCH:
        flush_wgrads()


def _wgrad_stream(dev):
    if not WGRAD_STREAM or dev.type != "cuda":
        return None
    from .streams import side_stream
    return side_stream(dev, _WGRAD_SIDE)


def _group_weights(weights, Cp, need_t):
    pre = [_prepped.get(w.data_ptr()) for w in weights] if _prepped else [None]
    if all(p is not None and (p[1] is not None or not need_t) for p in pre):
        wbs, wts = [p[0] for p in pre], [p[1] for p in pre]
        sb = _stride(wbs, 2)
        st = _stride(wts, 2) if need_t else 0
        n = wbs[0].numel()
        if sb is not None and st is not None and (len(wbs) == 1 or (abs(sb) >= n and (not need_t or abs(st) >= n))):
            return wbs[0], sb, wts[0], st
    lib = L.load()
    G = len(weights)
    K, C, R, S = weights[0].shape
    dev = weights[0].device
    wb = torch.empty(G, K, R, S, Cp, device=dev, dtype=BF)
    wt = torch.empty(G, Cp, R, S, K, device=dev, dtype=BF) if need_t else None
    for g, w in enumerate(weights):
        w32 = _nhwc(w.detach().float())
        L.check(lib.gm_conv_weight_prep_bf16(w32.data_ptr(), K, R * S, C, Cp, wb[g].data_ptr(),
                                             wt[g].data_ptr() if need_t else 0, L.stream_of(dev)),
                "gm_conv_weight_prep_bf16")
    n = K * R * S * Cp
    return wb[0], n, (wt[0] if need_t else None), n


class _VConvFn(torch.autograd.Function):

    @staticmethod
    def forward(ctx, X, G, stride, pad, join, stats, *weights):
        lib = L.load()
        ctx.join = join
        ctx.dlink = stats.get("dgrad_link") if stats is not None else None
        GN, C, H, W = X.shape
        N = GN // G
        K, C0, R, S = weights[0].shape
        if C != C0 or _cpad(C) != C or GN != N * G:
            raise L.GreedyMMLError(f"vtrunk conv: stacked input {tuple(X.shape)} does not fit {G} x {C0} channels")
        xb = _nhwc(X.to(BF))
        need_dx = ctx.needs_input_grad[0]
        wb, sb, wt, st = _group_weights(weights, C, need_dx)
        P = (H + 2 * pad - R) // stride + 1
        Q = (W + 2 * pad - S) // stride + 1
        y = torch.empty(GN, K, P, Q, device=X.device, dtype=BF, memory_format=CL)
        d = _desc_hw(N, H, W, C, K, R, S, stride, stride, pad, pad)
        ws, nb = _splitk_g(X.device, _desc(N, H, W, C, K, R, S, stride, pad), G, False)
        rc = _GM_E_UNSUP
        if stats is not None and EPI_BN_STATS and K % 64 == 0:
            nf = lib.gm_conv2d_fwd_bn_stats_floats(ctypes.byref(d), G)
            part = torch.empty(max(nf, 1), device=X.device, dtype=torch.float32)
            rows = ctypes.c_int(0)
            rc = lib.gm_conv2d_fwd_grouped_bn_stats_bf16(ctypes.byref(d), G, xb.data_ptr(), wb.data_ptr(), sb,
                                                         y.data_ptr(), part.data_ptr(), nf, ctypes.byref(rows), ws,
                                                         nb, L.stream_of(X.device))
            if rc == 0:
                stats["part"], stats["rows"] = part, rows.value
            elif rc != _GM_E_UNSUP:
                L.check(rc, "gm_conv2d_fwd_grouped_bn_stats_bf16")
        if rc != 0:
            L.check(lib.gm_conv2d_fwd_grouped_bf16(ctypes.byref(d), G, xb.data_ptr(), wb.data_ptr(), sb, y.data_ptr(),
                                                   ws, nb, L.stream_of(X.device)), "gm_conv2d_fwd_grouped_bf16")
        ctx.save_for_backward(xb, wt, *weights)
# ... 8 lines not shown
        GN, C, H, W = xb.shape
        K, _, R, S = weights[0].shape
        gy = _nhwc(gy.to(BF))
        dev = gy.device
        dx = None
        if ctx.needs_input_grad[0]:
            d = _desc(N, H, W, C, K, R, S, stride, pad)

            def dgrad(add):
                madd = add if isinstance(add, MaskedAddend) else None
                at = madd.dy if madd is not None else add
                if at is not None and (tuple(at.shape) != (GN, C, H, W) or at.dtype != BF
                                       or not at.is_contiguous(memory_format=CL)):
                    raise ValueError("vtrunk conv dgrad: addend must be bf16 channels_last shaped like dx")
                if madd is not None:
                    if madd.mask.numel() * 8 != at.numel():
                        raise ValueError("vtrunk conv dgrad: addend mask must hold one bit per element")
                    out = torch.empty(GN, C, H, W, device=dev, dtype=BF, memory_format=CL)
                    ws, nb = _splitk_g(dev, d, G, True)
                    L.check(lib.gm_conv2d_dgrad_grouped_masked_bf16(
                        ctypes.byref(d), G, gy.data_ptr(), wt.data_ptr(), st, out.data_ptr(), at.data_ptr(),
                        madd.mask.data_ptr(), ws, nb, L.stream_of(dev)), "gm_conv2d_dgrad_grouped_masked_bf16")
                    return out
                out = add if add is not None else torch.empty(GN, C, H, W, device=dev, dtype=BF, memory_format=CL)
                ws, nb = _splitk_g(dev, d, G, True)
                lk = ctx.dlink
                if add is None and lk is not None and "bn" in lk and EPI_BN_BWD_STATS:
                    bx, bcoef, bmean = lk.pop("bn")
                    if tuple(bx.shape) == (GN, C, H, W):
                        nf = lib.gm_conv2d_dgrad_bn_stats_floats(ctypes.byref(d), G)
                        part = torch.empty(max(nf, 1), device=dev, dtype=torch.float32)
                        rows = ctypes.c_int(0)
                        rc = lib.gm_conv2d_dgrad_grouped_bn_stats_bf16(
                            ctypes.byref(d), G, gy.data_ptr(), wt.data_ptr(), st, out.data_ptr(), bx.data_ptr(),
                            bcoef.data_ptr(), bmean.data_ptr(), part.data_ptr(), nf, ctypes.byref(rows), ws, nb,
                            L.stream_of(dev))
                        if rc == 0:
                            lk["part"], lk["rows"], lk["dy"] = part, rows.value, out
                            return out
                        if rc != _GM_E_UNSUP:
                            L.check(rc, "gm_conv2d_dgrad_grouped_bn_stats_bf16")
                L.check(lib.gm_conv2d_dgrad_grouped_bf16(ctypes.byref(d), G, gy.data_ptr(), wt.data_ptr(), st,
                                                         out.data_ptr(), L.ptr(add), ws, nb, L.stream_of(dev)),
                        "gm_conv2d_dgrad_grouped_bf16")
                return out
            dx = ctx.join.contribute(dgrad) if ctx.join is not None else dgrad(None)
        grads = [None] * G
        want = [ctx.needs_input_grad[6 + g] for g in range(G)]
        if any(want):
            dh = _desc_hw(N, H, W, C, K, R, S, stride, stride, pad, pad)
            tg = [sink_target(w) if wn else None for w, wn in zip(weights, want)]
            need = lib.gm_conv2d_wgrad_grouped_scratch(ctypes.byref(dh), G)
            scratch = torch.empty(max(need, 16), device=dev, dtype=torch.uint8)
            sunk = all(t is not None for t in tg)
            if sunk:
                bufs = [t[0] for t in tg]
                sd = _stride(bufs, 4)
                if (sd is None or len({t[1] for t in tg}) != 1 or (G > 1 and abs(sd) < bufs[0].numel())
                        or not all(b.is_contiguous(memory_format=CL) for b in bufs)):
                    raise RuntimeError("vtrunk conv: the views' gradient buffers must be channels_last, one "
                                       "accumulate state, at one stride (the engine's flat layout)")
                def launch(dh=dh, gy=gy, xb=xb, buf=bufs[0], sd=sd, acc=int(tg[0][1]), scratch=scratch, need=need):
                    L.check(lib.gm_conv2d_wgrad_grouped_bf16(ctypes.byref(dh), G, gy.data_ptr(), xb.data_ptr(),
                                                             buf.data_ptr(), sd, C, acc, scratch.data_ptr(), need,
                                                             L.stream_of(dev)), "gm_conv2d_wgrad_grouped_bf16")
                if _wgrad_stream(dev) is not None:
                    _defer_wgrad(launch, list(weights), (gy, xb, scratch), dev)
                else:
                    launch()
                    for w in weights:
                        sink_done(w)
            else:
                if any(t is not None for t in tg):
                    raise RuntimeError("vtrunk conv: all or none of the views' weights must be sink-managed")
                dw = torch.empty(G, K, R, S, C, device=dev, dtype=torch.float32)
                L.check(lib.gm_conv2d_wgrad_grouped_bf16(ctypes.byref(dh), G, gy.data_ptr(), xb.data_ptr(),
                                                         dw.data_ptr(), K * R * S * C, C, 0, scratch.data_ptr(),
                                                         need, L.stream_of(dev)), "gm_conv2d_wgrad_grouped_bf16")
                grads = [_like_param(dw[g].permute(0, 3, 1, 2), w) if wn else None
                         for g, (w, wn) in enumerate(zip(weights, want))]
        return (dx, None, None, None, None, None, *grads)


def vconv(X, convs, join=None, stats=None):
    c0 = convs[0]
    if not c0._hip_ok():
        raise L.GreedyMMLError("vtrunk conv: only the ResNet trunk's convolutions")
    if join is not None and X.requires_grad and torch.is_grad_enabled():
        join.register()
    else:
        join = None
    with torch.autocast("cuda", enabled=False):
        return _VConvFn.apply(X, len(convs), c0.stride[0], c0.padding[0], join, stats, *[c.weight for c in convs])



def _bn_param_grads(gammas, betas, want_w, want_b):
    G = len(gammas)
    tw = [sink_target(w) for w in gammas] if want_w and want_b else []
    tb = [sink_target(b) for b in betas] if want_w and want_b else []
    if tw and all(t is not None for t in tw + tb):
        accs = {t[1] for t in tw + tb}
        if len(accs) != 1:
            raise RuntimeError("vtrunk BatchNorm: the views' parameters must share one gradient sink state")
        return [t[0] for t in tw], [t[0] for t in tb], accs.pop(), True
    if any(t is not None for t in tw + tb):
        raise RuntimeError("vtrunk BatchNorm: all or none of the views' parameters must be sink-managed")
    C = gammas[0].shape[0]
    dev = gammas[0].device
    return ([torch.empty(C, device=dev, dtype=torch.float32) for _ in range(G)],
            [torch.empty(C, device=dev, dtype=torch.float32) for _ in range(G)], False, False)


def _bn_backward(dz, y, xb, G, gammas, betas, sm, si, relu, want_dres, coef, want_w, want_b, ymask=None):
    lib = L.load()
    GN, C, H, W = xb.shape
    M = (GN // G) * H * W
    dz = _nhwc(dz.to(BF))
    dx = torch.empty_like(xb, memory_format=CL)
    dres = torch.empty_like(xb, memory_format=CL) if want_dres else None
    dgs, dbs, acc, sunk = _bn_param_grads(gammas, betas, want_w, want_b)
    descs = []
    for g in range(G):
        r = slice(g * (GN // G), (g + 1) * (GN // G))
        descs.append(L.BnBwd(M, C, int(relu), dz[r].data_ptr(), y[r].data_ptr() if (relu and y is not None) else 0,
                             xb[r].data_ptr(), gammas[g].data_ptr(), sm[g].data_ptr(), si[g].data_ptr(),
                             dx[r].data_ptr(), dres[r].data_ptr() if dres is not None else 0, dgs[g].data_ptr(),
                             dbs[g].data_ptr(), int(acc), 0, coef[g].data_ptr() if coef is not None else 0,
                             ymask[g * (M * C // 8):].data_ptr() if ymask is not None else 0))
    buf = _bn_scratch_g(xb.device, M, C, G)
    L.check(lib.gm_bn_bwd_grouped_bf16(L.arr(L.BnBwd, descs), G, buf.data_ptr(), buf.numel(),
                                       L.stream_of(xb.device)), "gm_bn_bwd_grouped_bf16")
    if sunk:
        for p in list(gammas) + list(betas):
            sink_done(p)
        return dx, dres, [None] * G, [None] * G
    return dx, dres, [d if want_w else None for d in dgs], [d if want_b else None for d in dbs]


def _bn_backward_from_stats(dz, xb, G, gammas, betas, sm, si, coef, part, rows, want_w, want_b):
    lib = L.load()
    GN, C, H, W = xb.shape
    M = (GN // G) * H * W
    dx = torch.empty_like(xb, memory_format=CL)
    dgs, dbs, acc, sunk = _bn_param_grads(gammas, betas, want_w, want_b)
    descs = []
    for g in range(G):
        r = slice(g * (GN // G), (g + 1) * (GN // G))
        descs.append(L.BnBwd(M, C, 1, dz[r].data_ptr(), 0, xb[r].data_ptr(), gammas[g].data_ptr(),
                             sm[g].data_ptr(), si[g].data_ptr(), dx[r].data_ptr(), 0, dgs[g].data_ptr(),
                             dbs[g].data_ptr(), int(acc), 0, coef[g].data_ptr(), 0))
    st = L.stream_of(xb.device)
    arr = L.arr(L.BnBwd, descs)
    L.check(lib.gm_bn_bwd_stats_finalize_grouped(arr, G, part.data_ptr(), rows, st), "gm_bn_bwd_stats_finalize_grouped")
    L.check(lib.gm_bn_bwd_apply_grouped_bf16(arr, G, part.data_ptr(), rows, st), "gm_bn_bwd_apply_grouped_bf16")
    if sunk:
        for p in list(gammas) + list(betas):
            sink_done(p)
        return dx, [None] * G, [None] * G
    return dx, [d if want_w else None for d in dgs], [d if want_b else None for d in dbs]


class _VBNFn(torch.autograd.Function):

    @staticmethod
    def forward(ctx, X, residual, G, bns, relu, join, stats, *params):
        lib = L.load()
        ctx.join = join
        gammas, betas = params[:G], params[G:]
        xb = _nhwc(X.to(BF))
        GN, C, H, W = xb.shape
        N = GN // G
        M = N * H * W
        if residual is not None:
            residual = _nhwc(residual.to(BF))
        maskx = relu and residual is None and MASK_FROM_X
        y = torch.empty_like(xb, memory_format=CL)
        dev = xb.device
        sm = torch.empty(G, C, device=dev, dtype=torch.float32)
        si = torch.empty(G, C, device=dev, dtype=torch.float32)
        coef = torch.empty(G, 2 * C, device=dev, dtype=torch.float32) if maskx else None
        ymask = (torch.empty(GN * H * W * C // 8, device=dev, dtype=torch.uint8)
                 if relu and residual is not None and BN_RELU_MASK else None)
        descs = []
        for g, bn in enumerate(bns):
            r = slice(g * N, (g + 1) * N)
            descs.append(L.BnFwd(M, C, int(relu), xb[r].data_ptr(),
                                 residual[r].data_ptr() if residual is not None else 0, y[r].data_ptr(),
                                 gammas[g].data_ptr(), betas[g].data_ptr(), L.ptr(bn.running_mean),
                                 L.ptr(bn.running_var), float(bn.momentum), float(bn.eps), sm[g].data_ptr(),
                                 si[g].data_ptr(), L.ptr(bn.num_batches_tracked),
                                 coef[g].data_ptr() if maskx else 0,
                                 ymask[g * (M * C // 8):].data_ptr() if ymask is not None else 0))
        if stats is not None and "part" in stats:
            part, rows = stats.pop("part"), stats.pop("rows")
            st = L.stream_of(dev)
            L.check(lib.gm_bn_fwd_stats_finalize_grouped(L.arr(L.BnFwd, descs), G, part.data_ptr(), rows, st),
                    "gm_bn_fwd_stats_finalize_grouped")
            L.check(lib.gm_bn_fwd_apply_grouped_bf16(L.arr(L.BnFwd, descs), G, part.data_ptr(), rows, st),
                    "gm_bn_fwd_apply_grouped_bf16")
        else:
            buf = _bn_scratch_g(dev, M, C, G)
            L.check(lib.gm_bn_fwd_train_grouped_bf16(L.arr(L.BnFwd, descs), G, buf.data_ptr(), buf.numel(),
                                                     L.stream_of(dev)), "gm_bn_fwd_train_grouped_bf16")
        ctx.save_for_backward(xb, y if relu and not maskx else coef, sm, si, ymask, *gammas, *betas)
        ctx.meta = (G, maskx, relu, residual is not None)
        ctx.blink = stats.get("bn_link") if stats is not None else None
        ctx.rlink = stats.get("res_link") if stats is not None and ymask is not None else None
        ctx.zlink = stats.get("dz_link") if stats is not None and not relu and residual is None else None
        if ctx.blink is not None and maskx and G >= 2 and C % 64 == 0:
            ctx.blink["bn"] = (xb, coef, sm)
        return y

    @staticmethod
    def backward(ctx, dy):
        xb, yc, sm, si, ymask, *prm = ctx.saved_tensors
        G, maskx, relu, has_res = ctx.meta
        gammas, betas = prm[:G], prm[G:]
        y, coef = (None, yc) if maskx else (yc, None)
        want_dres = has_res and ctx.needs_input_grad[1]
        lk = ctx.blink
        want_w, want_b = any(ctx.needs_input_grad[7:7 + G]), any(ctx.needs_input_grad[7 + G:])
        if lk is not None and "part" in lk:
            part, rows, pdy = lk.pop("part"), lk.pop("rows"), lk.pop("dy")
            lk.pop("bn", None)
            if maskx and not want_dres and dy.data_ptr() == pdy.data_ptr() and dy.shape == pdy.shape:
                dx, gw, gb = _bn_backward_from_stats(pdy, xb, G, gammas, betas, sm, si, coef, part, rows,
                                                     want_w, want_b)
                return (dx if ctx.needs_input_grad[0] else None, None, None, None, None, None, None, *gw, *gb)
        zl = ctx.zlink
        if zl is not None and "dz" in zl:
            dyo, yo, mo = zl.pop("dz")
            if dy.data_ptr() != dyo.data_ptr() or dy.shape != dyo.shape:
                raise L.GreedyMMLError("vtrunk BatchNorm: the residual's gradient is not the block output's dy")
            dx, _, gw, gb = _bn_backward(dyo, yo, xb, G, gammas, betas, sm, si, True, False, None,
                                         want_w, want_b, mo)
            return (dx if ctx.needs_input_grad[0] else None, None, None, None, None, None, None, *gw, *gb)
        join = ctx.join
        if (want_dres and join is not None and ymask is not None and IDT_MASKED_ADDEND and join.masked_ok
                and join.first_of_many()):
            dyb = _nhwc(dy.to(BF))
            dx, _, gw, gb = _bn_backward(dyb, y, xb, G, gammas, betas, sm, si, relu, False, coef,
                                         want_w, want_b, ymask)
            join.contribute(lambda add: MaskedAddend(dyb, ymask))
            return (dx if ctx.needs_input_grad[0] else None, None, None, None, None, None, None, *gw, *gb)
        if want_dres and ctx.rlink is not None and DS_DZ_LINK:
            dyb = _nhwc(dy.to(BF))
            ctx.rlink["dz"] = (dyb, y, ymask)
            dx, _, gw, gb = _bn_backward(dyb, y, xb, G, gammas, betas, sm, si, relu, False, coef,
                                         want_w, want_b, ymask)
            return (dx if ctx.needs_input_grad[0] else None, dyb, None, None, None, None, None, *gw, *gb)
        dx, dres, gw, gb = _bn_backward(dy, y, xb, G, gammas, betas, sm, si, relu, want_dres, coef,
                                        want_w, want_b, ymask)
        if dres is not None and ctx.join is not None:
            dres = ctx.join.contribute(lambda add: dres if add is None else dres + add)
        return (dx if ctx.needs_input_grad[0] else None, dres, None, None, None, None, None, *gw, *gb)


def vbn(X, bns, residual=None, relu=False, residual_join=None, stats=None):
    b0 = bns[0]
    if any(b.momentum is None or b.momentum != b0.momentum or b.eps != b0.eps for b in bns):
        raise L.GreedyMMLError("vtrunk BatchNorm: the views must share momentum and eps")
    join = None
    if residual_join is not None and residual is not None and residual.requires_grad and torch.is_grad_enabled():
        residual_join.register()
        join = residual_join
    with torch.autocast("cuda", enabled=False):
        return _VBNFn.apply(X, residual, len(bns), bns, bool(relu), join, stats,
                            *[b.weight for b in bns], *[b.bias for b in bns])



class _VStemFn(torch.autograd.Function):

    @staticmethod
    def forward(ctx, x, G, pad, stats, *weights):
        lib = L.load()
        B, _, C0, H, W = x.shape
        K, _, R, S = weights[0].shape
        P, Q, Sp, Hp, Wp = _stem_geom(H, W, R, S, pad)
        dev = x.device
        xp = torch.empty(G * B, Hp, Wp // 2, 8, device=dev, dtype=BF)
        wp = torch.empty(G, K, R, Sp, 8, device=dev, dtype=BF)
        if G <= 4:
            stem_pack_grouped([x[:, g] for g in range(G)], weights, pad, xp, wp)
        else:
            for g in range(G):
                stem_pack(x[:, g], weights[g], pad, xp=xp[g * B:(g + 1) * B], wp=wp[g])
        y = torch.empty(G * B, K, P, Q, device=dev, dtype=BF, memory_format=CL)
        d = _desc_hw(B, Hp, Wp // 2, 8, K, R, Sp, 2, 1, 0, 0)
        rows = lib.gm_conv_stem_stats_rows(ctypes.byref(d), G) if (stats is not None and FUSED_STEM_STATS) else 0
        if rows > 0:
            part = torch.empty(G, rows + 1, 128, device=dev, dtype=torch.float32)
            L.check(lib.gm_conv2d_fwd_grouped_stats_bf16(ctypes.byref(d), G, xp.data_ptr(), wp.data_ptr(),
                                                         K * R * Sp * 8, y.data_ptr(), part.data_ptr(), rows,
                                                         L.stream_of(dev)), "gm_conv2d_fwd_grouped_stats_bf16")
            stats["part"], stats["rows"] = part, rows
        else:
            L.check(lib.gm_conv2d_fwd_grouped_bf16(ctypes.byref(d), G, xp.data_ptr(), wp.data_ptr(), K * R * Sp * 8,
                                                   y.data_ptr(), 0, 0, L.stream_of(dev)), "gm_conv2d_fwd_grouped_bf16")
        ctx.save_for_backward(xp, *weights)
        ctx.meta = (G, B, R, S, Sp)
        ctx.link = stats
        if stats is not None:
            stats["stem_bn_ok"] = FUSED_STEM_WGRAD and lib.gm_conv2d_wgrad_stem_bn_ok(ctypes.byref(d), G) == 1
        return y

    @staticmethod
    def backward(ctx, gy):
        xp, *weights = ctx.saved_tensors
        G, B, R, S, Sp = ctx.meta
        want = [ctx.needs_input_grad[4 + g] for g in range(G)]
        if not any(want):
            return (None, None, None, None, *[None] * G)
        lib = L.load()
        bw = ctx.link.pop("bwd", None) if ctx.link is not None else None
        if bw is None:
            gy = _nhwc(gy.to(BF))
        dev = gy.device
        _, Hp, Wq, _ = xp.shape
        K, C0 = weights[0].shape[0], weights[0].shape[1]
        d = _desc_hw(B, Hp, Wq, 8, K, R, Sp, 2, 1, 0, 0)
        need = lib.gm_conv2d_wgrad_grouped_scratch(ctypes.byref(d), G)
        scratch = torch.empty(max(need, 16), device=dev, dtype=torch.uint8)
        dwp = torch.empty(G, K, R, Sp, 8, device=dev, dtype=torch.float32)
        if bw is not None:
            src = L.StemBnSrc(bw["y"].data_ptr(), bw["dy_pool"].data_ptr(), bw["idx"].data_ptr(),
                              bw["fcoef"].data_ptr(), bw["fcoef"].stride(0), bw["bcoef"], bw["bcoef_gs"])
            L.check(lib.gm_conv2d_wgrad_stem_bn_grouped_bf16(ctypes.byref(d), G, ctypes.byref(src), xp.data_ptr(),
                                                             dwp.data_ptr(), K * R * Sp * 8, 0, scratch.data_ptr(),
                                                             need, L.stream_of(dev)),
                    "gm_conv2d_wgrad_stem_bn_grouped_bf16")
        else:
            L.check(lib.gm_conv2d_wgrad_grouped_bf16(ctypes.byref(d), G, gy.data_ptr(), xp.data_ptr(),
                                                     dwp.data_ptr(), K * R * Sp * 8, 8, 0, scratch.data_ptr(), need,
                                                     L.stream_of(dev)), "gm_conv2d_wgrad_grouped_bf16")
        tgts = [sink_target(w) if want[g] else None for g, w in enumerate(weights)]
        if all(t is not None and t[1] == tgts[0][1] and t[0].dtype == torch.float32
               and t[0].is_contiguous(memory_format=CL) for t in tgts):
            ptrs = (ctypes.c_void_p * G)(*[t[0].data_ptr() for t in tgts])
            L.check(lib.gm_stem_dw_crop(dwp.data_ptr(), G, K, R, S, C0, Sp, ptrs, int(bool(tgts[0][1])),
                                        L.stream_of(dev)), "gm_stem_dw_crop")
            for w in weights:
                sink_done(w)
            return (None, None, None, None, *[None] * G)
        grads = []
        for g, w in enumerate(weights):
            if not want[g]:
                grads.append(None)
                continue
            dw = dwp[g].view(K, R, 2 * Sp, 4)[:, :, :S, :C0].permute(0, 3, 1, 2)
            tgt = tgts[g]
            if tgt is not None:
                if tgt[1]:
                    tgt[0].add_(dw)
                else:
                    tgt[0].copy_(dw)
                sink_done(w)
                grads.append(None)
            else:
                grads.append(_like_param(dw, w))
        return (None, None, None, None, *grads)


class _VBNReluPoolFn(torch.autograd.Function):

    @staticmethod
    def forward(ctx, X, G, bns, k, s, pad, stats, *params):
        lib = L.load()
        gammas, betas = params[:G], params[G:]
        xb = _nhwc(X.to(BF))
        GN, C, H, W = xb.shape
        N = GN // G
        M = N * H * W
        dev = xb.device
        sm = torch.empty(G, C, device=dev, dtype=torch.float32)
        si = torch.empty(G, C, device=dev, dtype=torch.float32)
        coef = torch.empty(G, 2 * C, device=dev, dtype=torch.float32)
        descs = [L.BnFwd(M, C, 1, xb[g * N:(g + 1) * N].data_ptr(), 0, 0, gammas[g].data_ptr(), betas[g].data_ptr(),
                         L.ptr(bn.running_mean), L.ptr(bn.running_var), float(bn.momentum), float(bn.eps),
                         sm[g].data_ptr(), si[g].data_ptr(), L.ptr(bn.num_batches_tracked), coef[g].data_ptr())
                 for g, bn in enumerate(bns)]
        st = L.stream_of(dev)
        if stats is not None and "part" in stats:
            L.check(lib.gm_bn_fwd_stats_finalize_grouped(L.arr(L.BnFwd, descs), G, stats["part"].data_ptr(),
                                                         stats["rows"], st), "gm_bn_fwd_stats_finalize_grouped")
        else:
            buf = _bn_scratch_g(dev, M, C, G)
            L.check(lib.gm_bn_fwd_stats_grouped_bf16(L.arr(L.BnFwd, descs), G, buf.data_ptr(), buf.numel(), st),
                    "gm_bn_fwd_stats_grouped_bf16")
        P, Q = (H + 2 * pad - k) // s + 1, (W + 2 * pad - k) // s + 1
        y = torch.empty(GN, C, P, Q, device=dev, dtype=BF, memory_format=CL)
        idx = torch.empty(GN, P, Q, C, device=dev, dtype=torch.uint8)
        fused_bwd = FUSED_STEM_BWD and (k, s, pad, C) == (3, 2, 1, 64)
        xsel = torch.empty(GN, P, Q, C, device=dev, dtype=BF) if fused_bwd else None
        ctx.xsel_on = STEM_XSEL
        d = L.PoolDesc(N, H, W, C, k, s, pad)
        L.check(lib.gm_bn_relu_maxpool2d_fwd_grouped_bf16(ctypes.byref(d), G, xb.data_ptr(), coef.data_ptr(),
                                                          y.data_ptr(), idx.data_ptr(), L.ptr(xsel), st),
                "gm_bn_relu_maxpool2d_fwd_grouped_bf16")
        ctx.save_for_backward(xb, coef, sm, si, idx, xsel, *gammas, *betas)
        ctx.meta = (G, k, s, pad)
        ctx.link = stats
        return y

    @staticmethod
    def backward(ctx, dy):
        flush_wgrads()
        lib = L.load()
        xb, coef, sm, si, idx, xsel, *prm = ctx.saved_tensors
        G, k, s, pad = ctx.meta
        gammas, betas = prm[:G], prm[G:]
        GN, C, H, W = xb.shape
        dy = _nhwc(dy.to(BF))
        want_w, want_b = any(ctx.needs_input_grad[7:7 + G]), any(ctx.needs_input_grad[7 + G:])
        if xsel is not None and (want_w or want_b):
            N = GN // G
            M = N * H * W
            link = ctx.link if (ctx.needs_input_grad[0] and ctx.link is not None
                                and ctx.link.get("stem_bn_ok")) else None
            dx = None if link is not None else torch.empty_like(xb, memory_format=CL)
            dgs, dbs, acc, sunk = _bn_param_grads(gammas, betas, want_w, want_b)
            descs = [L.BnBwd(M, C, 1, 0, 0, xb[g * N:(g + 1) * N].data_ptr(), gammas[g].data_ptr(), sm[g].data_ptr(),
                             si[g].data_ptr(), dx[g * N:(g + 1) * N].data_ptr() if dx is not None else 0, 0,
                             dgs[g].data_ptr(), dbs[g].data_ptr(), int(acc), 0, coef[g].data_ptr())
                     for g in range(G)]
            buf = _bn_scratch_g(xb.device, M, C, G)
            d = L.PoolDesc(N, H, W, C, k, s, pad)
            if link is not None:
                bcoef, bgs = ctypes.c_void_p(), ctypes.c_longlong()
                L.check(lib.gm_bn_relu_maxpool2d_bwd_stats_grouped_bf16(
                    ctypes.byref(d), G, dy.data_ptr(), idx.data_ptr(), xsel.data_ptr() if ctx.xsel_on else 0,
                    L.arr(L.BnBwd, descs), buf.data_ptr(), buf.numel(), ctypes.byref(bcoef), ctypes.byref(bgs),
                    L.stream_of(xb.device)), "gm_bn_relu_maxpool2d_bwd_stats_grouped_bf16")
                link["bwd"] = dict(y=xb, dy_pool=dy, idx=idx, fcoef=coef, bcoef=bcoef.value, bcoef_gs=bgs.value,
                                   keep=buf)
                dx = torch.empty((), device=xb.device, dtype=xb.dtype).expand(xb.shape)
            else:
                L.check(lib.gm_bn_relu_maxpool2d_bwd_grouped_bf16(ctypes.byref(d), G, dy.data_ptr(), idx.data_ptr(),
                                                                  xsel.data_ptr() if ctx.xsel_on else 0,
                                                                  L.arr(L.BnBwd, descs), buf.data_ptr(),
                                                                  buf.numel(), L.stream_of(xb.device)),
                        "gm_bn_relu_maxpool2d_bwd_grouped_bf16")
            if sunk:
                for p in list(gammas) + list(betas):
                    sink_done(p)
                gw, gb = [None] * G, [None] * G
            else:
                gw = [t if want_w else None for t in dgs]
                gb = [t if want_b else None for t in dbs]
            return (dx if ctx.needs_input_grad[0] else None, None, None, None, None, None, None, *gw, *gb)
        dz = torch.empty_like(xb, memory_format=CL)
        d = L.PoolDesc(GN, H, W, C, k, s, pad)
        L.check(lib.gm_maxpool2d_bwd_bf16(ctypes.byref(d), dy.data_ptr(), idx.data_ptr(), dz.data_ptr(),
                                          L.stream_of(xb.device)), "gm_maxpool2d_bwd_bf16")
        dx, _, gw, gb = _bn_backward(dz, None, xb, G, gammas, betas, sm, si, True, False, coef, want_w, want_b)
        return (dx if ctx.needs_input_grad[0] else None, None, None, None, None, None, None, *gw, *gb)


def vstem(x, nets):
    G = len(nets)
    c0 = nets[0].conv1
    pool = nets[0].maxpool
    from .pool import _pair1
    k, s, p = (_pair1(getattr(pool, a)) for a in ("kernel_size", "stride", "padding"))
    stats = {}
    with torch.autocast("cuda", enabled=False):
        y = _VStemFn.apply(x, G, c0.padding[0], stats, *[n.conv1.weight for n in nets])
        bns = [n.bn1 for n in nets]
        return _VBNReluPoolFn.apply(y, G, bns, k, s, p, stats, *[b.weight for b in bns], *[b.bias for b in bns])



def vblock(blocks, X):
    b0 = blocks[0]
    join = GradJoin()
    ds = b0.downsample is not None
    join.masked_ok = not ds

    def cbn(x, convs, bns, cjoin=None, link_in=None, link_out=None, res_link=None, **kw):
        st = {"dgrad_link": link_in, "bn_link": link_out, "dz_link": res_link, "res_link": res_link}
        return vbn(vconv(x, convs, cjoin, stats=st), bns, stats=st, **kw)
    rl = {} if ds else None
    if ds:
        idt = cbn(X, [b.downsample[0] for b in blocks], [b.downsample[1] for b in blocks], join, res_link=rl)
    else:
        idt = X
    l1 = {}
    out = cbn(X, [b.conv1 for b in blocks], [b.bn1 for b in blocks], join, link_out=l1, relu=True)
    if hasattr(b0, "conv3"):
        l2 = {}
        out = cbn(out, [b.conv2 for b in blocks], [b.bn2 for b in blocks], link_in=l1, link_out=l2, relu=True)
        return cbn(out, [b.conv3 for b in blocks], [b.bn3 for b in blocks], link_in=l2, residual=idt, relu=True,
                   residual_join=None if ds else join, res_link=rl)
    return cbn(out, [b.conv2 for b in blocks], [b.bn2 for b in blocks], link_in=l1, residual=idt, relu=True,
               residual_join=None if ds else join, res_link=rl)


def vlayer(nets, i, X):
    layers = [getattr(n, f"layer{i}") for n in nets]
    for j in range(len(layers[0])):
        X = vblock([lay[j] for lay in layers], X)
    return X


def usable(model, nets, x):
    from .bn import GMBatchNorm2d
    from .conv import GMConv2d
    if not (ENABLED and model.training and x.is_cuda and x.dim() == 5 and 2 <= len(nets) <= 16):
        return False
    if not (x.dtype == BF or (torch.is_autocast_enabled("cuda") and torch.get_autocast_dtype("cuda") == BF)):
        return False
    if not torch.is_grad_enabled():
        return False
    sig = None
    for n in nets:
        if not n.training or not n.conv1.uses_pair_stem():
            return False
        mods = [m for m in n.modules() if isinstance(m, (GMConv2d, GMBatchNorm2d))]
        s = [(type(m).__name__, tuple(m.weight.shape)) for m in mods]
        if sig is None:
            sig = s
        elif s != sig:
            return False
        if any(isinstance(m, GMBatchNorm2d) and (m.momentum is None or not m.track_running_stats or not m.affine)
               for m in mods):
            return False
    return True



def vconv_affine(xb, G, wb, sb, K, R, S, stride, pad, area, residual=None, relu=True):
    lib = L.load()
    GN, C, H, W = xb.shape
    N = GN // G
    if GN != N * G or xb.dtype != BF or not xb.is_contiguous(memory_format=CL) or _cpad(C) != C:
        raise L.GreedyMMLError(f"vconv_affine: stacked bf16 channels_last input of {G} groups (got {tuple(xb.shape)})")
    if tuple(area.shape) != (G, 4 * K) or area.dtype != torch.float32 or not area.is_contiguous():
        raise L.GreedyMMLError("vconv_affine: coefficient area must be fp32 [G, 4K]")
    P, Q = (H + 2 * pad - R) // stride + 1, (W + 2 * pad - S) // stride + 1
    dev = xb.device
    y = torch.empty(GN, K, P, Q, device=dev, dtype=BF, memory_format=CL)
    if residual is not None and (residual.shape != y.shape or residual.dtype != BF
                                 or not residual.is_contiguous(memory_format=CL)):
        raise L.GreedyMMLError("vconv_affine: the residual must be bf16 channels_last shaped like the output")
    d = _desc_hw(N, H, W, C, K, R, S, stride, stride, pad, pad)
    ws, nb = _splitk_g(dev, _desc(N, H, W, C, K, R, S, stride, pad), G, False)
    st = L.stream_of(dev)
    if lib.gm_conv2d_fwd_affine_ok(ctypes.byref(d), G) == 1:
        L.check(lib.gm_conv2d_fwd_grouped_affine_bf16(ctypes.byref(d), G, xb.data_ptr(), wb.data_ptr(), sb,
                                                      y.data_ptr(), area.data_ptr() + 8 * K, 4 * K, L.ptr(residual),
                                                      int(bool(relu)), ws, nb, st),
                "gm_conv2d_fwd_grouped_affine_bf16")
        return y
    if K % 64:
        raise L.GreedyMMLError(f"vconv_affine: no kernel applies the coefficients for K = {K}")
    L.check(lib.gm_conv2d_fwd_grouped_bf16(ctypes.byref(d), G, xb.data_ptr(), wb.data_ptr(), sb, y.data_ptr(), ws, nb,
                                           st), "gm_conv2d_fwd_grouped_bf16")
    a = area.data_ptr()
    descs = [L.BnFwd(N * P * Q, K, int(bool(relu)), y[g * N:(g + 1) * N].data_ptr(),
                     residual[g * N:(g + 1) * N].data_ptr() if residual is not None else 0,
                     y[g * N:(g + 1) * N].data_ptr(), a, a, 0, 0, 0.0, 0.0, a, a, 0, 0, 0) for g in range(G)]
    L.check(lib.gm_bn_fwd_apply_grouped_bf16(L.arr(L.BnFwd, descs), G, a, 1, st), "gm_bn_fwd_apply_grouped_bf16")
    return y


class _EvalPos:

    def __init__(self, convs, bns):
        self.convs, self.bns = convs, bns
        self.K, self.C, self.R, self.S = convs[0].weight.shape
        self.stride, self.pad = convs[0].stride[0], convs[0].padding[0]
        self.wb = self.area = None


class EvalTrunk:

    def __init__(self, nets):
        from .bn import GMBatchNorm2d
        from .conv import GMConv2d
        self.nets = list(nets)
        self.G = G = len(self.nets)
        if not 2 <= G <= 16:
            raise L.GreedyMMLError("EvalTrunk: 2..16 views")
        sig = None
        for n in self.nets:
            mods = [m for m in n.modules() if isinstance(m, (GMConv2d, GMBatchNorm2d))]
            s = [(type(m).__name__, tuple(m.weight.shape)) for m in mods]
            if sig is not None and s != sig:
                raise L.GreedyMMLError("EvalTrunk: the views must share one architecture")
            sig = s
            if not n.conv1.uses_pair_stem() or any(
                    isinstance(m, GMBatchNorm2d) and (not m.track_running_stats or not m.affine) for m in mods):
                raise L.GreedyMMLError("EvalTrunk: pixel-pair stem, affine BatchNorms with running statistics")
        n0 = self.nets[0]
        self.stem_bns = [n.bn1 for n in self.nets]
        self.blocks = {}
        self.pos = []
        for i in (1, 2, 3, 4):
            layers = [getattr(n, f"layer{i}") for n in self.nets]
            blks = []
            for j in range(len(layers[0])):
                bs = [lay[j] for lay in layers]
                e = {}
                for k in (1, 2, 3):
                    if hasattr(bs[0], f"conv{k}"):
                        e[f"conv{k}"] = _EvalPos([getattr(b, f"conv{k}") for b in bs], [getattr(b, f"bn{k}") for b in bs])
                if bs[0].downsample is not None:
                    e["ds"] = _EvalPos([b.downsample[0] for b in bs], [b.downsample[1] for b in bs])
                for p in e.values():
                    if not p.convs[0]._hip_ok() or _cpad(p.C) != p.C or p.K % 64:
                        raise L.GreedyMMLError("EvalTrunk: only the ResNet trunk's convolutions")
                self.pos.extend(e.values())
                blks.append(e)
            self.blocks[i] = blks
        from .pool import _pair1
        self.pool = tuple(_pair1(getattr(n0.maxpool, a)) for a in ("kernel_size", "stride", "padding"))
        self.coef = self.stem_coef = self._table = self._idx = None
        self._n_entries = self._max_c = 0

    def refresh(self):
        lib = L.load()
        G = self.G
        dev = self.nets[0].conv1.weight.device
        st = L.stream_of(dev)
        if self.coef is None or self.coef.device != dev:
            Cs = self.stem_bns[0].weight.shape[0]
            total = G * 2 * Cs + sum(G * 4 * p.K for p in self.pos)
            self.coef = torch.zeros(total, device=dev, dtype=torch.float32)
            self.stem_coef = self.coef[:G * 2 * Cs].view(G, 2 * Cs)
            off = G * 2 * Cs
            for p in self.pos:
                p.area = self.coef[off:off + G * 4 * p.K].view(G, 4 * p.K)
                off += G * 4 * p.K
                p.wb = torch.empty(G, p.K, p.R, p.S, p.C, device=dev, dtype=BF)
        ents = []

        def entry(bn, out_ptr):
            if bn.running_mean is None or bn.running_mean.dtype != torch.float32 or bn.weight.dtype != torch.float32:
                raise L.GreedyMMLError("EvalTrunk: fp32 BatchNorm parameters and running statistics")
            ents.append(L.BnCoefEntry(bn.weight.data_ptr(), bn.bias.data_ptr(), bn.running_mean.data_ptr(),
                                      bn.running_var.data_ptr(), out_ptr, bn.weight.shape[0], float(bn.eps)))
        for g, bn in enumerate(self.stem_bns):
            entry(bn, self.stem_coef[g].data_ptr())
        for p in self.pos:
            for g, bn in enumerate(p.bns):
                entry(bn, p.area[g].data_ptr() + 8 * p.K)
        raw = bytes(L.arr(L.BnCoefEntry, ents))
        if self._table is None or self._table.device != dev or self._table.numel() != len(raw):
# ... 161 lines not shown
```

include/greedymml.h:

```cpp
#ifndef GREEDYMML_H
#define GREEDYMML_H

#include <stddef.h>
#include <stdint.h>

#ifdef __cplusplus
extern "C" {
#endif

#define GM_ABI_VERSION 5

#define GM_F32  0
#define GM_BF16 1
#define GM_NCHW 0
#define GM_NHWC 1
#define GM_OK          0
#define GM_E_ARG      -1
#define GM_E_SCRATCH  -2
#define GM_E_UNSUP    -3

int gm_abi_version(void);
const char* gm_last_error(void);

#define GM_FAULT_BN_SPIN     1u
// ... 169 lines not shown
int gm_conv_set_rw(int on);
int gm_conv_set_stem(int on);
int gm_conv_set_wgrad_stem(int on);
int gm_conv2d_fwd_ex_bf16(const gm_conv_desc* d, const void* x, const void* w, void* y, void* ws,
                          size_t ws_bytes, void* stream);
int gm_conv2d_dgrad_ex_bf16(const gm_conv_desc* d, const void* dy, const void* wt, void* dx, void* ws,
                            size_t ws_bytes, void* stream);
int gm_conv2d_dgrad_add_bf16(const gm_conv_desc* d, const void* dy, const void* wt, void* dx,
                             const void* addend, void* ws, size_t ws_bytes, void* stream);
int gm_conv_weight_transpose_bf16(const void* w, void* wt, int K, int RS, int C, void* stream);
int gm_conv_weight_prep_bf16(const float* w, int K, int RS, int C, int Cp, void* wb, void* wt, void* stream);
typedef struct gm_wprep {
    const float* w;
    void* wb;
    void* wt;
    int K, RS, C, Cp;
    int tile_start;
    int pad;
} gm_wprep;
int gm_wprep_tiles(int K, int RS, int Cp);
int gm_conv_weight_prep_multi_bf16(const gm_wprep* table, int n, int total_tiles, void* stream);
size_t gm_conv2d_wgrad_scratch(const gm_conv_desc* d);
int gm_conv2d_wgrad_bf16(const gm_conv_desc* d, const void* dy, const void* x, float* dw, int c_real,
                         int accumulate, void* scratch, size_t scratch_bytes, void* stream);
size_t gm_conv2d_wgrad_hw_scratch(const gm_conv_desc_hw* d);
int gm_conv2d_wgrad_hw_bf16(const gm_conv_desc_hw* d, const void* dy, const void* x, float* dw, int c_real,
                            int accumulate, void* scratch, size_t scratch_bytes, void* stream);
int gm_conv2d_fwd_grouped_bf16(const gm_conv_desc_hw* d, int G, const void* x, const void* w, long long w_stride,
                               void* y, void* ws, size_t ws_bytes, void* stream);
int gm_conv2d_dgrad_grouped_bf16(const gm_conv_desc* d, int G, const void* dy, const void* wt, long long wt_stride,
                                 void* dx, const void* addend, void* ws, size_t ws_bytes, void* stream);
int gm_conv2d_dgrad_grouped_masked_bf16(const gm_conv_desc* d, int G, const void* dy, const void* wt,
                                        long long wt_stride, void* dx, const void* addend, const void* addend_mask,
                                        void* ws, size_t ws_bytes, void* stream);
size_t gm_conv2d_splitk_ws_bytes_grouped(const gm_conv_desc* d, int G, int dgrad);
size_t gm_conv2d_wgrad_grouped_scratch(const gm_conv_desc_hw* d, int G);
int gm_conv2d_wgrad_grouped_bf16(const gm_conv_desc_hw* d, int G, const void* dy, const void* x, float* dw,
                                 long long dw_stride, int c_real, int accumulate, void* scratch,
                                 size_t scratch_bytes, void* stream);
typedef struct gm_stem_bn_src {
    const void* y;
    const void* dy_pool;
    const void* idx;
    const float* fcoef;
    long long fcoef_gs;
    const float* bcoef;
    long long bcoef_gs;
} gm_stem_bn_src;
int gm_stem_dw_crop(const float* dwp, int G, int K, int R, int S, int C0, int Sp, float* const* dst, int accumulate,
                    void* stream);
int gm_conv2d_wgrad_stem_bn_ok(const gm_conv_desc_hw* d, int G);
int gm_conv2d_wgrad_stem_bn_grouped_bf16(const gm_conv_desc_hw* d, int G, const gm_stem_bn_src* src, const void* x,
                                         float* dw, long long dw_stride, int accumulate, void* scratch,
                                         size_t scratch_bytes, void* stream);

#define GM_CONV_FWD   0
#define GM_CONV_DGRAD 1
#define GM_CONV_WGRAD 2
typedef struct gm_conv_f32 {
    int mode;
    gm_conv_desc d;
    const float* x;
    const float* w;
    const float* dy;
    float* out;
    const float* addend;
    int accumulate;
    int pad0;
} gm_conv_f32;

size_t gm_conv2d_f32_scratch(const gm_conv_f32* p);
int gm_conv2d_f32(const gm_conv_f32* p, void* scratch, size_t scratch_bytes, void* stream);

size_t gm_conv2d_f32_split_scratch(const gm_conv_f32* p, int terms);
int gm_conv2d_f32_split(const gm_conv_f32* p, int terms, void* scratch, size_t scratch_bytes, void* stream);

int gm_conv2d_f32_affine(const gm_conv_f32* p, int terms, const float* coef, const float* residual, int relu,
                         void* scratch, size_t scratch_bytes, void* stream);

typedef struct gm_bn_fwd {
    long long M;
    int C, relu;
    const void* x;
    const void* residual;
    void* y;
    const float* gamma;
    const float* beta;
    float* running_mean;
    float* running_var;
    float momentum, eps;
    float* save_mean;
    float* save_invstd;
    long long* num_batches_tracked;
    float* coef_out;
    void* relu_mask;
} gm_bn_fwd;

typedef struct gm_bn_bwd {
    long long M;
    int C, relu;
    const void* dy;
    const void* y;
    const void* x;
    const float* gamma;
    const float* save_mean;
    const float* save_invstd;
    void* dx;
    void* dres;
    float* dgamma;
    float* dbeta;
    int accumulate;
    int pad;
    const float* fwd_coef;
    const void* relu_mask;
} gm_bn_bwd;

size_t gm_bn_scratch(long long M, int C);
int gm_bn_fwd_train_bf16(const gm_bn_fwd* p, void* scratch, size_t scratch_bytes, void* stream);
int gm_bn_fwd_infer_bf16(const gm_bn_fwd* p, void* scratch, size_t scratch_bytes, void* stream);
int gm_bn_bwd_bf16(const gm_bn_bwd* p, void* scratch, size_t scratch_bytes, void* stream);
int gm_bn_fwd_stats_bf16(const gm_bn_fwd* p, void* scratch, size_t scratch_bytes, void* stream);
size_t gm_bn_scratch_grouped(long long M, int C, int G);
int gm_bn_fwd_train_grouped_bf16(const gm_bn_fwd* ps, int G, void* scratch, size_t scratch_bytes, void* stream);
int gm_bn_bwd_grouped_bf16(const gm_bn_bwd* ps, int G, void* scratch, size_t scratch_bytes, void* stream);
int gm_bn_fwd_stats_grouped_bf16(const gm_bn_fwd* ps, int G, void* scratch, size_t scratch_bytes, void* stream);
int gm_bn_fwd_train_f32(const gm_bn_fwd* p, void* scratch, size_t scratch_bytes, void* stream);
int gm_bn_fwd_infer_f32(const gm_bn_fwd* p, void* scratch, size_t scratch_bytes, void* stream);
int gm_bn_bwd_f32(const gm_bn_bwd* p, void* scratch, size_t scratch_bytes, void* stream);

typedef struct gm_pool_desc {
    int N, H, W, C;
    int k, stride, pad;
} gm_pool_desc;

int gm_maxpool2d_fwd_bf16(const gm_pool_desc* d, const void* x, void* y, void* idx, void* stream);
int gm_maxpool2d_bwd_bf16(const gm_pool_desc* d, const void* dy, const void* idx, void* dx, void* stream);
int gm_conv_stem_stats_rows(const gm_conv_desc_hw* d, int G);
int gm_conv2d_fwd_grouped_stats_bf16(const gm_conv_desc_hw* d, int G, const void* x, const void* w,
                                     long long w_stride, void* y, float* stats, int rows, void* stream);
int gm_bn_fwd_stats_finalize_grouped(const gm_bn_fwd* ps, int G, float* stats, int rows, void* stream);
size_t gm_conv2d_fwd_bn_stats_floats(const gm_conv_desc_hw* d, int G);
int gm_conv2d_fwd_grouped_bn_stats_bf16(const gm_conv_desc_hw* d, int G, const void* x, const void* w,
                                        long long w_stride, void* y, float* stats, size_t stats_floats,
                                        int* rows_out, void* ws, size_t ws_bytes, void* stream);
int gm_bn_fwd_apply_grouped_bf16(const gm_bn_fwd* ps, int G, const float* stats, int rows, void* stream);
size_t gm_conv2d_dgrad_bn_stats_floats(const gm_conv_desc* d, int G);
int gm_conv2d_dgrad_grouped_bn_stats_bf16(const gm_conv_desc* d, int G, const void* dy, const void* wt,
                                          long long wt_stride, void* dx, const void* bn_x, const float* bn_coef,
                                          const float* bn_mean, float* stats, size_t stats_floats, int* rows_out,
                                          void* ws, size_t ws_bytes, void* stream);
size_t gm_bn_bwd_stats_coef_offset(int C, int G, int rows);
int gm_bn_bwd_stats_finalize_grouped(const gm_bn_bwd* ps, int G, float* stats, int rows, void* stream);
int gm_bn_bwd_apply_grouped_bf16(const gm_bn_bwd* ps, int G, const float* stats, int rows, void* stream);
int gm_bn_relu_maxpool2d_bwd_grouped_bf16(const gm_pool_desc* d, int G, const void* dy_pool, const void* idx,
                                          const void* xsel, const gm_bn_bwd* ps, void* scratch, size_t scratch_bytes,
                                          void* stream);
int gm_bn_relu_maxpool2d_bwd_stats_grouped_bf16(const gm_pool_desc* d, int G, const void* dy_pool, const void* idx,
                                                const void* xsel, const gm_bn_bwd* ps, void* scratch,
                                                size_t scratch_bytes, const float** bcoef, long long* bcoef_gs,
                                                void* stream);
int gm_bn_relu_maxpool2d_fwd_bf16(const gm_pool_desc* d, const void* x, const float* coef, void* y, void* idx,
                                  void* stream);
int gm_bn_relu_maxpool2d_fwd_grouped_bf16(const gm_pool_desc* d, int G, const void* x, const float* coef, void* y,
                                          void* idx, void* xsel, void* stream);
int gm_maxpool2d_fwd_f32(const gm_pool_desc* d, const void* x, void* y, void* idx, void* stream);
int gm_maxpool2d_bwd_f32(const gm_pool_desc* d, const void* dy, const void* idx, void* dx, void* stream);

typedef struct gm_views_norm {
    const uint8_t* x;
    const uint8_t* flip;
    int B, V, H, W, C;
    float mean[4], std[4];
    void* out;
    int dtype, layout;
} gm_views_norm;

int gm_views_normalize(const gm_views_norm* p, void* stream);

typedef struct {
    const float* gamma;
    const float* beta;
    const float* running_mean;
    const float* running_var;
    float* coef;
    int C;
    float eps;
} gm_bn_coef_entry;

int gm_bn_infer_coef(const gm_bn_coef_entry* table, int n, int max_c, void* stream);
int gm_conv2d_fwd_affine_ok(const gm_conv_desc_hw* d, int G);
int gm_conv2d_fwd_grouped_affine_bf16(const gm_conv_desc_hw* d, int G, const void* x, const void* w,
                                      long long w_stride, void* y, const float* coef, long long coef_stride,
                                      const void* residual, int relu, void* ws, size_t ws_bytes, void* stream);
int gm_eval_metrics(const float* logits, int nbranch, int B, int N, const long long* labels, void* acc,
                    void* stream);

#ifdef __cplusplus
}
#endif
#endif
```

Measured before the change: 36780 view-images/s.

## Fuse BatchNorm stats finalize with apply, and fold downsample BN into block output

Adds kernels that combine the BN statistics-finalize step with the normalize/apply pass, in both forward and backward. Each block recomputes the per-channel coefficients redundantly from the partial sums and then streams the activations, so one launch and one round trip of the coefficients are removed. A second path fuses the downsample branch's BN as a residual affine into the block output BN kernel, so the normalized identity tensor is never materialized. In exchange, every block redoes the partial-sum reduction, the code grows, and the new path is gated behind flags.

```diff
diff --git a/greedy_multimodal_learning_amd/_lib.py b/greedy_multimodal_learning_amd/_lib.py
--- a/greedy_multimodal_learning_amd/_lib.py
+++ b/greedy_multimodal_learning_amd/_lib.py
@@ -280,6 +280,15 @@
     "gm_bn_bwd_stats_coef_offset": (c_size_t, [c_int, c_int, c_int]),
     "gm_bn_bwd_stats_finalize_grouped": (c_int, [c_void_p, c_int, c_void_p, c_int, c_void_p]),
     "gm_bn_bwd_apply_grouped_bf16": (c_int, [c_void_p, c_int, c_void_p, c_int, c_void_p]),
+    "gm_bn_fold_blocks": (c_int, [ctypes.c_longlong, c_int, c_int, c_int]),
+    "gm_bn_fwd_finalize_apply_grouped_bf16": (c_int, [c_void_p, c_int, c_void_p, c_int, c_void_p]),
+    "gm_bn_fwd_finalize_apply_grouped_bf16_ex": (c_int, [c_void_p, c_int, c_void_p, c_int, c_int, c_void_p]),
+    "gm_bn_bwd_finalize_apply_grouped_bf16": (c_int, [c_void_p, c_int, c_void_p, c_int, c_void_p]),
+    "gm_bn_bwd_finalize_apply_grouped_bf16_ex": (c_int, [c_void_p, c_int, c_void_p, c_int, c_int, c_void_p]),
+    "gm_bn_fwd_finalize_apply_res_affine_grouped_bf16": (c_int, [c_void_p, c_int, c_void_p, c_int, c_void_p,
+                                                                 c_void_p, c_int, c_void_p]),
+    "gm_bn_fwd_finalize_apply_res_affine_grouped_bf16_ex": (c_int, [c_void_p, c_int, c_void_p, c_int, c_void_p,
+                                                                    c_void_p, c_int, c_int, c_void_p]),
     "gm_maxpool2d_bwd_bf16": (c_int, [c_void_p, c_void_p, c_void_p, c_void_p, c_void_p]),
 })
 
diff --git a/greedy_multimodal_learning_amd/csrc/batchnorm.hip b/greedy_multimodal_learning_amd/csrc/batchnorm.hip
--- a/greedy_multimodal_learning_amd/csrc/batchnorm.hip
+++ b/greedy_multimodal_learning_amd/csrc/batchnorm.hip
@@ -274,62 +274,101 @@
     return f;
 }
 
+struct FwdCoef {
+    float sc, sh, mean, invstd, rmean, rvar;
+};
+struct BwdCoef {
+    float ca, cb, cc, c3, dg, db;
+};
+
+__device__ __forceinline__ FwdCoef fwd_coef(const ReduceArgs& a, double S1, double S2, double invM, const FinOps& f) {
+    FwdCoef k;
+    const double g = (double)f.g;
+    const double mean = S1 * invM;
+    double var = S2 * invM - mean * mean;
+    if (var < 0.0) var = 0.0;
+    const double invstd = 1.0 / sqrt(var + (double)a.eps);
+    const double sc = g * invstd;
+    k.sc = (float)sc;
+    k.sh = (float)((double)f.b - mean * sc);
+    k.mean = (float)mean;
+    k.invstd = (float)invstd;
+    const double m = (double)a.momentum;
+    const double unb = a.M > 1 ? var * (double)a.M / (double)(a.M - 1) : var;
+    k.rmean = (float)((1.0 - m) * (double)f.rm + m * mean);
+    k.rvar = (float)((1.0 - m) * (double)f.rv + m * unb);
+    return k;
+}
+
+template <bool CENTER>
+__device__ __forceinline__ BwdCoef bwd_coef(double S1, double S2, double invM, const FinOps& f) {
+    BwdCoef k;
+    const double g = (double)f.g;
+    const double mean = (double)f.rm;
+    const double is = (double)f.rv;
+    const double ca = g * is;
+    const double cb = -g * is * is * is * S2 * invM;
+    k.ca = (float)ca;
+    k.cb = (float)cb;
+    if (CENTER) {
+        k.cc = (float)(-ca * S1 * invM);
+        k.c3 = (float)mean;
+    } else {
+        k.cc = (float)(-ca * S1 * invM - cb * mean);
+        k.c3 = 0.f;
+    }
+    k.dg = (float)(S2 * is);
+    k.db = (float)S1;
+    return k;
+}
+
+template <bool SC1>
+__device__ __forceinline__ void fwd_store(const ReduceArgs& a, int c, const FwdCoef& k) {
+    const int C = a.C;
+    a.coef[c] = k.sc;
+    a.coef[C + c] = k.sh;
+    if (SC1) {
+        st_sc1(&a.coef[c], k.sc);
+        st_sc1(&a.coef[C + c], k.sh);
+    }
+    if (a.coef_out) {
+        a.coef_out[c] = k.sc;
+        a.coef_out[C + c] = k.sh;
+    }
+    a.save_mean[c] = k.mean;
+    a.save_invstd[c] = k.invstd;
+    if (a.rmean) {
+        a.rmean[c] = k.rmean;
+        a.rvar[c] = k.rvar;
+    }
+}
+
+template <bool SC1, bool CENTER>
+__device__ __forceinline__ void bwd_store(const ReduceArgs& a, int c, const BwdCoef& k) {
+    const int C = a.C;
+    a.coef[c] = k.ca;
+    a.coef[C + c] = k.cb;
+    a.coef[2 * C + c] = k.cc;
+    if (CENTER) a.coef[3 * C + c] = k.c3;
+    if (SC1) {
+        st_sc1(&a.coef[c], k.ca);
+        st_sc1(&a.coef[C + c], k.cb);
+        st_sc1(&a.coef[2 * C + c], k.cc);
+    }
+    if (a.accumulate) {
+        a.dgamma[c] += k.dg;
+        a.dbeta[c] += k.db;
+    } else {
+        a.dgamma[c] = k.dg;
+        a.dbeta[c] = k.db;
+    }
+}
+
 template <int MODE, bool SC1 = false, bool CENTER = false>
 __device__ __forceinline__ void finalize(const ReduceArgs& a, int c, double S1, double S2, double invM,
                                          const FinOps& f) {
-    const int C = a.C;
-    const double g = (double)f.g;
-    if (MODE == FWD) {
-        const double mean = S1 * invM;
-        double var = S2 * invM - mean * mean;
-        if (var < 0.0) var = 0.0;
-        const double invstd = 1.0 / sqrt(var + (double)a.eps);
-        const double sc = g * invstd;
-        a.coef[c] = (float)sc;
-        a.coef[C + c] = (float)((double)f.b - mean * sc);
-        if (SC1) {
-            st_sc1(&a.coef[c], a.coef[c]);
-            st_sc1(&a.coef[C + c], a.coef[C + c]);
-        }
-        if (a.coef_out) {
-            a.coef_out[c] = a.coef[c];
-            a.coef_out[C + c] = a.coef[C + c];
-        }
-        a.save_mean[c] = (float)mean;
-        a.save_invstd[c] = (float)invstd;
-        if (a.rmean) {
-            const double m = (double)a.momentum;
-            const double unb = a.M > 1 ? var * (double)a.M / (double)(a.M - 1) : var;
-            a.rmean[c] = (float)((1.0 - m) * (double)f.rm + m * mean);
-            a.rvar[c] = (float)((1.0 - m) * (double)f.rv + m * unb);
-        }
-    } else {
-        const double mean = (double)f.rm;
-        const double is = (double)f.rv;
-        const double ca = g * is;
-        const double cb = -g * is * is * is * S2 * invM;
-        a.coef[c] = (float)ca;
-        a.coef[C + c] = (float)cb;
-        if (CENTER) {
-            a.coef[2 * C + c] = (float)(-ca * S1 * invM);
-            a.coef[3 * C + c] = (float)mean;
-        } else {
-            a.coef[2 * C + c] = (float)(-ca * S1 * invM - cb * mean);
-        }
-        if (SC1) {
-            st_sc1(&a.coef[c], a.coef[c]);
-            st_sc1(&a.coef[C + c], a.coef[C + c]);
-            st_sc1(&a.coef[2 * C + c], a.coef[2 * C + c]);
-        }
-        const float dg = (float)(S2 * is), db = (float)S1;
-        if (a.accumulate) {
-            a.dgamma[c] += dg;
-            a.dbeta[c] += db;
-        } else {
-            a.dgamma[c] = dg;
-            a.dbeta[c] = db;
-        }
-    }
+    if (MODE == FWD) fwd_store<SC1>(a, c, fwd_coef(a, S1, S2, invM, f));
+    else bwd_store<SC1, CENTER>(a, c, bwd_coef<CENTER>(S1, S2, invM, f));
 }
 
 
@@ -660,41 +699,61 @@
 }
 
 constexpr int kFinT = 1024;
+__device__ __forceinline__ void load_coef(const float* p, int cg, float* c);
+
+__device__ __forceinline__ void res_affine(float* r, const float* sc, const float* sh) {
+#pragma unroll
+    for (int j = 0; j < 8; ++j) r[j] = fmaf(r[j], sc[j], sh[j]);
+    unpack8(pack8(r), r);
+}
+
+__device__ __forceinline__ void fin_combine(const ReduceArgs& a, int cs, double (*rd)[128], double& S1, double& S2) {
+    const int t = threadIdx.x;
+    const int lv = t & 31, rg = t >> 5;
+    const float4* rows = reinterpret_cast<const float4*>(a.part + (size_t)cs * a.nrc * 128);
+    double d0 = 0.0, d1 = 0.0, d2 = 0.0, d3 = 0.0;
+    for (int i0 = rg; i0 < a.nrc; i0 += 8 * 32) {
+        float4 v[8];
+#pragma unroll
+        for (int u = 0; u < 8; ++u) v[u] = rows[(size_t)min(i0 + u * 32, a.nrc - 1) * 32 + lv];
+#pragma unroll
+        for (int u = 0; u < 8; ++u) {
+            if (i0 + u * 32 >= a.nrc) v[u] = make_float4(0.f, 0.f, 0.f, 0.f);
+            d0 += (double)v[u].x; d1 += (double)v[u].y; d2 += (double)v[u].z; d3 += (double)v[u].w;
+        }
+    }
+    rd[rg][4 * lv] = d0; rd[rg][4 * lv + 1] = d1; rd[rg][4 * lv + 2] = d2; rd[rg][4 * lv + 3] = d3;
+    __syncthreads();
+    S1 = 0.0;
+    S2 = 0.0;
+    if (t < 64) {
+        for (int i = 0; i < kFinT / 32; ++i) {
+            S1 += rd[i][2 * t];
+            S2 += rd[i][2 * t + 1];
+        }
+    }
+}
+
+__device__ __forceinline__ FinOps fin_load_fwd_all(const ReduceArgs& a, int cs) {
+    FinOps fo;
+    const int c = cs * 64 + (threadIdx.x & 63);
+    const float* rm = a.rmean ? a.rmean : a.gamma;
+    const float* rv = a.rmean ? a.rvar : a.gamma;
+    fo.g = a.gamma[c];
+    fo.b = a.beta[c];
+    fo.rm = rm[c];
+    fo.rv = rv[c];
+    return fo;
+}
+
 __global__ __launch_bounds__(kFinT) void k_bn_stats_finalize(ReduceArgs a0) {
     const ReduceArgs a = group_args(a0);
     __shared__ double rd[kFinT / 32][128];
     const int t = threadIdx.x, cs = blockIdx.y;
-    const int lv = t & 31, rg = t >> 5;
-    FinOps fo;
-    {
-        const int c = cs * 64 + (t & 63);
-        const float* rm = a.rmean ? a.rmean : a.gamma;
-        const float* rv = a.rmean ? a.rvar : a.gamma;
-        fo.g = a.gamma[c];
-        fo.b = a.beta[c];
-        fo.rm = rm[c];
-        fo.rv = rv[c];
-    }
-    const float4* rows = reinterpret_cast<const float4*>(a.part + (size_t)cs * a.nrc * 128);
-    double d0 = 0.0, d1 = 0.0, d2 = 0.0, d3 = 0.0;
-    for (int i0 = rg; i0 < a.nrc; i0 += 8 * 32) {
-        float4 v[8];
-#pragma unroll
-        for (int u = 0; u < 8; ++u) v[u] = rows[(size_t)min(i0 + u * 32, a.nrc - 1) * 32 + lv];
-#pragma unroll
-        for (int u = 0; u < 8; ++u) {
-            if (i0 + u * 32 >= a.nrc) v[u] = make_float4(0.f, 0.f, 0.f, 0.f);
-            d0 += (double)v[u].x; d1 += (double)v[u].y; d2 += (double)v[u].z; d3 += (double)v[u].w;
-        }
-    }
-    rd[rg][4 * lv] = d0; rd[rg][4 * lv + 1] = d1; rd[rg][4 * lv + 2] = d2; rd[rg][4 * lv + 3] = d3;
-    __syncthreads();
+    const FinOps fo = fin_load_fwd_all(a, cs);
+    double S1, S2;
+    fin_combine(a, cs, rd, S1, S2);
     if (t < 64) {
-        double S1 = 0.0, S2 = 0.0;
-        for (int i = 0; i < kFinT / 32; ++i) {
-            S1 += rd[i][2 * t];
-            S2 += rd[i][2 * t + 1];
-        }
         finalize<FWD>(a, cs * 64 + t, S1, S2, 1.0 / (double)a.M, fo);
         if (a.nbt && cs == 0 && t == 0) *a.nbt += 1;
     }
@@ -705,29 +764,206 @@
     a.coef = coef0 + blockIdx.z * cstride;
     __shared__ double rd[kFinT / 32][128];
     const int t = threadIdx.x, cs = blockIdx.y;
-    const int lv = t & 31, rg = t >> 5;
     const FinOps fo = fin_load<BWD>(a, cs * 64 + (t & 63));
-    const float4* rows = reinterpret_cast<const float4*>(a.part + (size_t)cs * a.nrc * 128);
-    double d0 = 0.0, d1 = 0.0, d2 = 0.0, d3 = 0.0;
-    for (int i0 = rg; i0 < a.nrc; i0 += 8 * 32) {
-        float4 v[8];
-#pragma unroll
-        for (int u = 0; u < 8; ++u) v[u] = rows[(size_t)min(i0 + u * 32, a.nrc - 1) * 32 + lv];
-#pragma unroll
-        for (int u = 0; u < 8; ++u) {
-            if (i0 + u * 32 >= a.nrc) v[u] = make_float4(0.f, 0.f, 0.f, 0.f);
-            d0 += (double)v[u].x; d1 += (double)v[u].y; d2 += (double)v[u].z; d3 += (double)v[u].w;
-        }
-    }
-    rd[rg][4 * lv] = d0; rd[rg][4 * lv + 1] = d1; rd[rg][4 * lv + 2] = d2; rd[rg][4 * lv + 3] = d3;
+    double S1, S2;
+    fin_combine(a, cs, rd, S1, S2);
+    if (t < 64) finalize<BWD>(a, cs * 64 + t, S1, S2, 1.0 / (double)a.M, fo);
+}
+
+struct ResBn {
+    int nrc;
+    float momentum, eps;
+    float* part;
+    unsigned long long scr_stride;
+    struct Grp {
+        const float* gamma;
+        const float* beta;
+        float* rmean;
+        float* rvar;
+        float* save_mean;
+        float* save_invstd;
+        long long* nbt;
+        float* coef_out;
+    } grp[kMaxBnG];
+};
+
+__device__ __forceinline__ ReduceArgs res_bn_args(const ReduceArgs& a, const ResBn& rb) {
+    ReduceArgs r = a;
+    const ResBn::Grp& q = rb.grp[blockIdx.z];
+    r.nrc = rb.nrc; r.momentum = rb.momentum; r.eps = rb.eps;
+    r.part = reinterpret_cast<float*>(reinterpret_cast<char*>(rb.part) + blockIdx.z * rb.scr_stride);
+    r.coef = r.part + (size_t)rb.nrc * 2 * a.C;
+    r.gamma = q.gamma; r.beta = q.beta; r.rmean = q.rmean; r.rvar = q.rvar;
+    r.save_mean = q.save_mean; r.save_invstd = q.save_invstd; r.nbt = q.nbt; r.coef_out = q.coef_out;
+    return r;
+}
+
+template <bool RES, bool RELU, bool RAFF>
+__device__ __forceinline__ void finalize_apply_body(const ReduceArgs& a0, const ResBn* rb) {
+    const ReduceArgs a = group_args(a0);
+    __shared__ double rd[kFinT / 32][128];
+    __shared__ float cf[RAFF ? 4 : 2][64];
+    const int t = threadIdx.x, cs = blockIdx.y;
+    const FinOps fo = fin_load_fwd_all(a, cs);
+    double S1, S2;
+    fin_combine(a, cs, rd, S1, S2);
+    if (t < 64) {
+        const FwdCoef k = fwd_coef(a, S1, S2, 1.0 / (double)a.M, fo);
+        cf[0][t] = k.sc;
+        cf[1][t] = k.sh;
+        if (blockIdx.x == 0) {
+            fwd_store<false>(a, cs * 64 + t, k);
+            if (a.nbt && cs == 0 && t == 0) *a.nbt += 1;
+        }
+    }
     __syncthreads();
+    if (RAFF) {
+        const ReduceArgs ar = res_bn_args(a, *rb);
+        const FinOps fr = fin_load_fwd_all(ar, cs);
+        fin_combine(ar, cs, rd, S1, S2);
+        if (t < 64) {
+            const FwdCoef k = fwd_coef(ar, S1, S2, 1.0 / (double)ar.M, fr);
+            cf[2][t] = k.sc;
+            cf[3][t] = k.sh;
+            if (blockIdx.x == 0) {
+                fwd_store<false>(ar, cs * 64 + t, k);
+                if (ar.nbt && cs == 0 && t == 0) *ar.nbt += 1;
+            }
+        }
+        __syncthreads();
+    }
+    const int j8 = (t & 7) * 8;
+    float sc[8], sh[8], rsc[8], rsh[8];
+#pragma unroll
+    for (int j = 0; j < 8; ++j) {
+        sc[j] = cf[0][j8 + j];
+        sh[j] = cf[1][j8 + j];
+        if (RAFF) {
+            rsc[j] = cf[2][j8 + j];
+            rsh[j] = cf[3][j8 + j];
+        }
+    }
+    typedef unsigned u32x4 __attribute__((ext_vector_type(4)));
+    const unsigned vpr = (unsigned)a.C >> 3, M = (unsigned)a.M;
+    const u32x4* XX = static_cast<const u32x4*>(a.x) + cs * 8;
+    const u32x4* RR = reinterpret_cast<const u32x4*>(a.res) + cs * 8;
+    uint4* YY = a.yout + cs * 8;
+    uint8_t* MM = a.mask_out ? a.mask_out + cs * 8 : nullptr;
+    auto fin = [&](unsigned i, u32x4 wx, u32x4 wr) {
+        float f[8], r[8];
+        unpack8(make_uint4(wx.x, wx.y, wx.z, wx.w), f);
+        if (RES) unpack8(make_uint4(wr.x, wr.y, wr.z, wr.w), r);
+        if (RAFF) res_affine(r, rsc, rsh);
+#pragma unroll
+        for (int j = 0; j < 8; ++j) {
+            float z = fmaf(f[j], sc[j], sh[j]);
+            if (RES) z += r[j];
+            f[j] = RELU ? relu_nan(z) : z;
+        }
+        const uint4 o = pack8(f);
+        YY[i] = o;
+        if (RES && RELU && MM) MM[i] = (uint8_t)mask_byte(o);
+    };
+    constexpr unsigned U = 4;
+    const unsigned st = gridDim.x * (kFinT / 8);
+    unsigned p = blockIdx.x * (kFinT / 8) + (t >> 3);
+    const unsigned lane = t & 7;
+    for (; p < M; p += U * st) {
+        u32x4 rx[U], rr[U];
+#pragma unroll
+        for (unsigned u = 0; u < U; ++u) {
+            const unsigned q = p + u * st < M ? p + u * st : p;
+            rx[u] = XX[q * vpr + lane];
+            if (RES) rr[u] = RR[q * vpr + lane];
+        }
+#pragma unroll
+        for (unsigned u = 0; u < U; ++u) {
+            asm volatile("" : "+v"(rx[u]));
+            if (RES) asm volatile("" : "+v"(rr[u]));
+        }
+#pragma unroll
+        for (unsigned u = 0; u < U; ++u)
+            if (p + u * st < M) fin((p + u * st) * vpr + lane, rx[u], RES ? rr[u] : rx[u]);
+    }
+}
+
+template <bool RES, bool RELU>
+__global__ __launch_bounds__(kFinT) void k_bn_finalize_apply(ReduceArgs a0) {
+    finalize_apply_body<RES, RELU, false>(a0, nullptr);
+}
+
+template <bool RELU>
+__global__ __launch_bounds__(kFinT) void k_bn_finalize_apply_raff(ReduceArgs a0, ResBn rb) {
+    finalize_apply_body<true, RELU, true>(a0, &rb);
+}
+
+template <bool RELU>
+__global__ __launch_bounds__(kFinT) void k_bn_bwd_finalize_apply(ReduceArgs a0, float* coef0, long long cstride) {
+    ReduceArgs a = group_args(a0);
+    a.coef = coef0 + blockIdx.z * cstride;
+    __shared__ double rd[kFinT / 32][128];
+    __shared__ float cf[3][64];
+    const int t = threadIdx.x, cs = blockIdx.y;
+    const FinOps fo = fin_load<BWD>(a, cs * 64 + (t & 63));
+    const int j8 = (t & 7) * 8;
+    double S1, S2;
+    fin_combine(a, cs, rd, S1, S2);
+    float fs[8], fh[8];
+    if (RELU) {
+        load_coef(a.fcoef, cs * 8 + (t & 7), fs);
+        load_coef(a.fcoef + a.C, cs * 8 + (t & 7), fh);
+    }
     if (t < 64) {
-        double S1 = 0.0, S2 = 0.0;
-        for (int i = 0; i < kFinT / 32; ++i) {
-            S1 += rd[i][2 * t];
-            S2 += rd[i][2 * t + 1];
-        }
-        finalize<BWD>(a, cs * 64 + t, S1, S2, 1.0 / (double)a.M, fo);
+        const BwdCoef k = bwd_coef<false>(S1, S2, 1.0 / (double)a.M, fo);
+        cf[0][t] = k.ca;
+        cf[1][t] = k.cb;
+        cf[2][t] = k.cc;
+        if (blockIdx.x == 0) bwd_store<false, false>(a, cs * 64 + t, k);
+    }
+    __syncthreads();
+    float ca[8], cb[8], cc[8];
+#pragma unroll
+    for (int j = 0; j < 8; ++j) {
+        ca[j] = cf[0][j8 + j];
+        cb[j] = cf[1][j8 + j];
+        cc[j] = cf[2][j8 + j];
+    }
+    typedef unsigned u32x4 __attribute__((ext_vector_type(4)));
+    const unsigned vpr = (unsigned)a.C >> 3, M = (unsigned)a.M;
+    const u32x4* DY = static_cast<const u32x4*>(a.dy) + cs * 8;
+    const u32x4* XX = static_cast<const u32x4*>(a.x) + cs * 8;
+    uint4* DX = a.yout + cs * 8;
+    auto out = [&](unsigned i, u32x4 wd, u32x4 wx) {
+        float d[8], xf[8], o[8];
+        unpack8(make_uint4(wd.x, wd.y, wd.z, wd.w), d);
+        unpack8(make_uint4(wx.x, wx.y, wx.z, wx.w), xf);
+        if (RELU) {
+#pragma unroll
+            for (int j = 0; j < 8; ++j) d[j] = fmaf(xf[j], fs[j], fh[j]) > 0.f ? d[j] : 0.f;
+        }
+#pragma unroll
+        for (int j = 0; j < 8; ++j) o[j] = fmaf(ca[j], d[j], fmaf(cb[j], xf[j], cc[j]));
+        DX[i] = pack8(o);
+    };
+    constexpr unsigned U = 4;
+    const unsigned st = gridDim.x * (kFinT / 8);
+    unsigned p = blockIdx.x * (kFinT / 8) + (t >> 3);
+    const unsigned lane = t & 7;
+    for (; p < M; p += U * st) {
+        u32x4 rdy[U], rx[U];
+#pragma unroll
+        for (unsigned u = 0; u < U; ++u) {
+            const unsigned q = p + u * st < M ? p + u * st : p;
+            rdy[u] = DY[q * vpr + lane];
+            rx[u] = XX[q * vpr + lane];
+        }
+#pragma unroll
+        for (unsigned u = 0; u < U; ++u) asm volatile("" : "+v"(rdy[u]), "+v"(rx[u]));
+#pragma unroll
+        for (unsigned u = 0; u < U; ++u) {
+            if (p + u * st < M) out((p + u * st) * vpr + lane, rdy[u], rx[u]);
+            __builtin_amdgcn_sched_barrier(0);
+        }
     }
 }
 
@@ -1251,6 +1487,8 @@
     long long cgs;
     long long fcgs;
     uint8_t* mask_out;
+    const float* rcoef;
+    long long rcgs;
 };
 
 __device__ __forceinline__ void load_coef(const float* p, int cg, float* c) {
@@ -1259,7 +1497,7 @@
     c[0] = a.x; c[1] = a.y; c[2] = a.z; c[3] = a.w; c[4] = b.x; c[5] = b.y; c[6] = b.z; c[7] = b.w;
 }
 
-template <bool RES, bool RELU, typename E>
+template <bool RES, bool RELU, typename E, bool RAFF = false>
 __global__ __launch_bounds__(kT) void k_bn_apply(ApplyArgs a) {
     const long long stride = (long long)gridDim.x * kT;
     long long v = (long long)blockIdx.x * kT + threadIdx.x;
@@ -1269,7 +1507,13 @@
     float sc[8], sh[8];
     load_coef(coef, cg, sc);
     load_coef(coef + a.C, cg, sh);
-    auto fin = [&](long long i, float* f, const float* r) {
+    float rsc[8], rsh[8];
+    if (RAFF) {
+        load_coef(a.rcoef + blockIdx.y * a.rcgs, cg, rsc);
+        load_coef(a.rcoef + blockIdx.y * a.rcgs + a.C, cg, rsh);
+    }
+    auto fin = [&](long long i, float* f, float* r) {
+        if (RAFF) res_affine(r, rsc, rsh);
 #pragma unroll
         for (int j = 0; j < 8; ++j) {
             float z = fmaf(f[j], sc[j], sh[j]);
@@ -1973,6 +2217,48 @@
     return stem_pool_bwd(d, G, dy_pool, idx, xsel, ps, scratch, bytes, false, bcoef, bcoef_gs, stream, fn);
 }
 
+static void fwd_stats_args(gm::ReduceArgs& a, const gm_bn_fwd* ps, int G, float* stats, int rows) {
+    const int C = ps[0].C;
+    a.M = ps[0].M; a.C = C; a.SW = 64; a.tpr_log = 3; a.nrc = rows;
+    a.momentum = ps[0].momentum; a.eps = ps[0].eps;
+    a.part = stats;
+    a.coef = stats + (size_t)rows * 2 * C;
+    a.scr_stride = (unsigned long long)(rows + 1) * 2 * C * sizeof(float);
+    a.hdr_words = 0;
+    for (int g = 0; g < G; ++g) {
+        gm::BnGroup& q = a.grp[g];
+        q.x = ps[g].x;
+        q.gamma = ps[g].gamma; q.beta = ps[g].beta;
+        q.rmean = ps[g].running_mean; q.rvar = ps[g].running_var;
+        q.save_mean = ps[g].save_mean; q.save_invstd = ps[g].save_invstd;
+        q.nbt = ps[g].num_batches_tracked;
+        q.coef_out = ps[g].coef_out;
+        q.res = static_cast<const uint4*>(ps[g].residual);
+        q.yout = static_cast<uint4*>(ps[g].y);
+        q.mask_out = static_cast<uint8_t*>(ps[g].relu_mask);
+    }
+}
+
+static void bwd_stats_args(gm::ReduceArgs& a, const gm_bn_bwd* ps, int G, float* stats, int rows) {
+    const int C = ps[0].C;
+    a.M = ps[0].M; a.C = C; a.SW = 64; a.tpr_log = 3; a.nrc = rows;
+    a.accumulate = ps[0].accumulate;
+    a.part = stats;
+    a.coef = stats;
+    a.scr_stride = (unsigned long long)(rows + 1) * 2 * C * sizeof(float);
+    a.hdr_words = 0;
+    for (int g = 0; g < G; ++g) {
+        gm::BnGroup& q = a.grp[g];
+        q.x = ps[g].x; q.dy = ps[g].dy;
+        q.gamma = ps[g].gamma;
+        q.save_mean = const_cast<float*>(ps[g].save_mean);
+        q.save_invstd = const_cast<float*>(ps[g].save_invstd);
+        q.dgamma = ps[g].dgamma; q.dbeta = ps[g].dbeta;
+        q.fcoef = ps[g].fwd_coef;
+        q.yout = static_cast<uint4*>(ps[g].dx);
+    }
+}
+
 extern "C" int gm_bn_fwd_stats_finalize_grouped(const gm_bn_fwd* ps, int G, float* stats, int rows, void* stream) {
     const char* fn = "gm_bn_fwd_stats_finalize_grouped";
     int rc = check_groups_fwd(ps, G, fn);
@@ -1981,27 +2267,13 @@
     GM_REQUIRE(stats && rows >= 1 && C >= 64 && C % 64 == 0 && ps[0].M >= 1, "%s: C a multiple of 64, rows >= 1",
                fn);
     ReduceArgs a{};
-    a.M = ps[0].M; a.C = C; a.SW = 64; a.tpr_log = 3; a.nrc = rows;
-    a.momentum = ps[0].momentum; a.eps = ps[0].eps;
-    a.part = stats;
-    a.coef = stats + (size_t)rows * 2 * C;
-    a.scr_stride = (unsigned long long)(rows + 1) * 2 * C * sizeof(float);
-    a.hdr_words = 0;
-    for (int g = 0; g < G; ++g) {
-        BnGroup& q = a.grp[g];
-        q.x = ps[g].x;
-        q.gamma = ps[g].gamma; q.beta = ps[g].beta;
-        q.rmean = ps[g].running_mean; q.rvar = ps[g].running_var;
-        q.save_mean = ps[g].save_mean; q.save_invstd = ps[g].save_invstd;
-        q.nbt = ps[g].num_batches_tracked;
-        q.coef_out = ps[g].coef_out;
-    }
+    fwd_stats_args(a, ps, G, stats, rows);
     hipLaunchKernelGGL(k_bn_stats_finalize, dim3(1, C / 64, G), dim3(kFinT), 0, as_stream(stream), a);
     return check_launch("k_bn_stats_finalize");
 }
 
-extern "C" int gm_bn_fwd_apply_grouped_bf16(const gm_bn_fwd* ps, int G, const float* stats, int rows, void* stream) {
-    const char* fn = "gm_bn_fwd_apply_grouped_bf16";
+static int fwd_apply(const gm_bn_fwd* ps, int G, const float* stats, int rows, const float* rstats, int rrows,
+                     void* stream, const char* fn) {
     int rc = check_groups_fwd(ps, G, fn);
     if (rc) return rc;
     const gm_bn_fwd* p = ps;
@@ -2028,7 +2300,13 @@
         b.gvec = strided ? gs / 8 : 0;
         b.cgs = strided ? cgs : 0;
         const dim3 g(apply_grid(b.nvec, C), strided ? G : 1);
-        if (p->residual) {
+        if (rstats) {
+            const long long rcgs = (long long)(rrows + 1) * 2 * C;
+            b.rcoef = rstats + gi * rcgs + (size_t)rrows * 2 * C;
+            b.rcgs = strided ? rcgs : 0;
+            if (p->relu) hipLaunchKernelGGL((k_bn_apply<true, true, uint16_t, true>), g, dim3(kT), 0, st, b);
+            else hipLaunchKernelGGL((k_bn_apply<true, false, uint16_t, true>), g, dim3(kT), 0, st, b);
+        } else if (p->residual) {
             if (p->relu) hipLaunchKernelGGL((k_bn_apply<true, true, uint16_t>), g, dim3(kT), 0, st, b);
             else hipLaunchKernelGGL((k_bn_apply<true, false, uint16_t>), g, dim3(kT), 0, st, b);
         } else {
@@ -2038,6 +2316,10 @@
         if ((rc = check_launch("k_bn_apply"))) return rc;
     }
     return GM_OK;
+}
+
+extern "C" int gm_bn_fwd_apply_grouped_bf16(const gm_bn_fwd* ps, int G, const float* stats, int rows, void* stream) {
+    return fwd_apply(ps, G, stats, rows, nullptr, 0, stream, "gm_bn_fwd_apply_grouped_bf16");
 }
 
 extern "C" size_t gm_bn_bwd_stats_coef_offset(int C, int G, int rows) {
@@ -2061,20 +2343,7 @@
     if (rc) return rc;
     const int C = ps[0].C;
     ReduceArgs a{};
-    a.M = ps[0].M; a.C = C; a.SW = 64; a.tpr_log = 3; a.nrc = rows;
-    a.accumulate = ps[0].accumulate;
-    a.part = stats;
-    a.coef = stats;
-    a.scr_stride = (unsigned long long)(rows + 1) * 2 * C * sizeof(float);
-    a.hdr_words = 0;
-    for (int g = 0; g < G; ++g) {
-        BnGroup& q = a.grp[g];
-        q.x = ps[g].x; q.dy = ps[g].dy;
-        q.gamma = ps[g].gamma;
-        q.save_mean = const_cast<float*>(ps[g].save_mean);
-        q.save_invstd = const_cast<float*>(ps[g].save_invstd);
-        q.dgamma = ps[g].dgamma; q.dbeta = ps[g].dbeta;
-    }
+    bwd_stats_args(a, ps, G, stats, rows);
     float* coef0 = stats + gm_bn_bwd_stats_coef_offset(C, G, rows);
     hipLaunchKernelGGL(k_bn_bwd_stats_finalize, dim3(1, C / 64, G), dim3(kFinT), 0, as_stream(stream), a, coef0,
                        (long long)4 * C);
@@ -2114,3 +2383,136 @@
     }
     return GM_OK;
 }
+
+constexpr int kFoldGrid = 256;
+constexpr int kFoldMaxRows = 1024;
+constexpr int kFoldReread = 2;
+constexpr long long kFoldMaxElems = 1ll << 25;
+
+extern "C" int gm_bn_fold_blocks(long long M, int C, int rows, int G) {
+    if (M < 1 || rows < 1 || rows > kFoldMaxRows || C < 64 || C % 64 != 0 || G < 1) return 0;
+    if (M * C >= (1ll << 31)) return 0;
+    if (M * C * G > kFoldMaxElems) return 0;
+    long long nb = kFoldGrid / ((long long)(C / 64) * G);
+    if (nb < 1) nb = 1;
+    const long long by_pixels = (M + 255) / 256;
+    if (nb > by_pixels) nb = by_pixels;
+    const long long by_reread = (long long)kFoldReread * M * 256 / ((long long)rows * 512);
+    if (nb > by_reread) nb = by_reread;
+    return nb < 1 ? 0 : (int)nb;
+}
+
+static int fold_nb_arg(long long M, int C, int rows, int G, int nb, const char* fn) {
+    GM_REQUIRE(nb >= 0 && nb <= 65535, "%s: nb in 0 (the rule) .. 65535 (got %d)", fn, nb);
+    GM_REQUIRE(nb == 0 || M * C < (1ll << 31), "%s: nb > 0 needs M * C < 2^31", fn);
+    return nb > 0 ? nb : gm_bn_fold_blocks(M, C, rows, G);
+}
+
+extern "C" int gm_bn_fwd_finalize_apply_grouped_bf16_ex(const gm_bn_fwd* ps, int G, float* stats, int rows, int nb,
+                                                        void* stream) {
+    const char* fn = "gm_bn_fwd_finalize_apply_grouped_bf16_ex";
+    int rc = check_groups_fwd(ps, G, fn);
+    if (rc) return rc;
+    const int C = ps[0].C;
+    GM_REQUIRE(stats && rows >= 1 && C >= 64 && C % 64 == 0 && ps[0].M >= 1 && ps[0].y,
+               "%s: C a multiple of 64, rows >= 1, y", fn);
+    for (int g = 0; g < G; ++g)
+        GM_REQUIRE(!ps[g].relu_mask == !ps[0].relu_mask, "%s: relu_mask in all groups or none", fn);
+    nb = fold_nb_arg(ps[0].M, C, rows, G, nb, fn);
+    if (nb < 0) return nb;
+    if (nb == 0) {
+        if ((rc = gm_bn_fwd_stats_finalize_grouped(ps, G, stats, rows, stream))) return rc;
+        return gm_bn_fwd_apply_grouped_bf16(ps, G, stats, rows, stream);
+    }
+    ReduceArgs a{};
+    fwd_stats_args(a, ps, G, stats, rows);
+    const dim3 grid(nb, C / 64, G), blk(kFinT);
+    hipStream_t st = as_stream(stream);
+    if (ps[0].residual) {
+        if (ps[0].relu) hipLaunchKernelGGL((k_bn_finalize_apply<true, true>), grid, blk, 0, st, a);
+        else hipLaunchKernelGGL((k_bn_finalize_apply<true, false>), grid, blk, 0, st, a);
+    } else {
+        if (ps[0].relu) hipLaunchKernelGGL((k_bn_finalize_apply<false, true>), grid, blk, 0, st, a);
+        else hipLaunchKernelGGL((k_bn_finalize_apply<false, false>), grid, blk, 0, st, a);
+    }
+    return check_launch("k_bn_finalize_apply");
+}
+
+extern "C" int gm_bn_fwd_finalize_apply_grouped_bf16(const gm_bn_fwd* ps, int G, float* stats, int rows, void* stream) {
+    return gm_bn_fwd_finalize_apply_grouped_bf16_ex(ps, G, stats, rows, 0, stream);
+}
+
+extern "C" int gm_bn_fwd_finalize_apply_res_affine_grouped_bf16_ex(const gm_bn_fwd* ps, int G, float* stats, int rows,
+                                                                   const gm_bn_fwd* rps, float* rstats, int rrows,
+                                                                   int nb, void* stream) {
+    const char* fn = "gm_bn_fwd_finalize_apply_res_affine_grouped_bf16_ex";
+    int rc = check_groups_fwd(ps, G, fn);
+    if (rc || (rc = check_groups_fwd(rps, G, fn))) return rc;
+    const int C = ps[0].C;
+    GM_REQUIRE(stats && rstats && rows >= 1 && rrows >= 1 && C >= 64 && C % 64 == 0 && ps[0].M >= 1 && ps[0].y,
+               "%s: C a multiple of 64, rows >= 1, y", fn);
+    for (int g = 0; g < G; ++g) {
+        GM_REQUIRE(!ps[g].relu_mask == !ps[0].relu_mask, "%s: relu_mask in all groups or none", fn);
+        GM_REQUIRE(ps[g].residual && rps[g].x == ps[g].residual && rps[g].M == ps[0].M && rps[g].C == C &&
+                       !rps[g].relu && !rps[g].residual,
+                   "%s: group %d: the residual must be its BatchNorm's input (same shape, no ReLU, no residual)",
+                   fn, g);
+    }
+    nb = fold_nb_arg(ps[0].M, C, rows + rrows, G, nb, fn);
+    if (nb < 0) return nb;
+    if (nb == 0) {
+        if ((rc = gm_bn_fwd_stats_finalize_grouped(ps, G, stats, rows, stream))) return rc;
+        if ((rc = gm_bn_fwd_stats_finalize_grouped(rps, G, rstats, rrows, stream))) return rc;
+        return fwd_apply(ps, G, stats, rows, rstats, rrows, stream, fn);
+    }
+    ReduceArgs a{};
+    fwd_stats_args(a, ps, G, stats, rows);
+    ResBn rb{};
+    rb.nrc = rrows; rb.momentum = rps[0].momentum; rb.eps = rps[0].eps;
+    rb.part = rstats;
+    rb.scr_stride = (unsigned long long)(rrows + 1) * 2 * C * sizeof(float);
+    for (int g = 0; g < G; ++g) {
+        ResBn::Grp& q = rb.grp[g];
+        q.gamma = rps[g].gamma; q.beta = rps[g].beta;
+        q.rmean = rps[g].running_mean; q.rvar = rps[g].running_var;
+        q.save_mean = rps[g].save_mean; q.save_invstd = rps[g].save_invstd;
+        q.nbt = rps[g].num_batches_tracked; q.coef_out = rps[g].coef_out;
+    }
+    const dim3 grid(nb, C / 64, G), blk(kFinT);
+    hipStream_t st = as_stream(stream);
+    if (ps[0].relu) hipLaunchKernelGGL(k_bn_finalize_apply_raff<true>, grid, blk, 0, st, a, rb);
+    else hipLaunchKernelGGL(k_bn_finalize_apply_raff<false>, grid, blk, 0, st, a, rb);
+    return check_launch("k_bn_finalize_apply_raff");
+}
+
+extern "C" int gm_bn_fwd_finalize_apply_res_affine_grouped_bf16(const gm_bn_fwd* ps, int G, float* stats, int rows,
+                                                                const gm_bn_fwd* rps, float* rstats, int rrows,
+                                                                void* stream) {
+    return gm_bn_fwd_finalize_apply_res_affine_grouped_bf16_ex(ps, G, stats, rows, rps, rstats, rrows, 0, stream);
+}
+
+extern "C" int gm_bn_bwd_finalize_apply_grouped_bf16_ex(const gm_bn_bwd* ps, int G, float* stats, int rows, int nb,
+                                                        void* stream) {
+    const char* fn = "gm_bn_bwd_finalize_apply_grouped_bf16_ex";
+    int rc = check_bwd_from_stats(ps, G, stats, rows, fn);
+    if (rc) return rc;
+    const int C = ps[0].C;
+    nb = fold_nb_arg(ps[0].M, C, rows, G, nb, fn);
+    if (nb < 0) return nb;
+    if (nb == 0) {
+        if ((rc = gm_bn_bwd_stats_finalize_grouped(ps, G, stats, rows, stream))) return rc;
+        return gm_bn_bwd_apply_grouped_bf16(ps, G, stats, rows, stream);
+    }
+    ReduceArgs a{};
+    bwd_stats_args(a, ps, G, stats, rows);
+    float* coef0 = stats + gm_bn_bwd_stats_coef_offset(C, G, rows);
+    const dim3 grid(nb, C / 64, G), blk(kFinT);
+    hipStream_t st = as_stream(stream);
+    if (ps[0].relu) hipLaunchKernelGGL(k_bn_bwd_finalize_apply<true>, grid, blk, 0, st, a, coef0, (long long)4 * C);
+    else hipLaunchKernelGGL(k_bn_bwd_finalize_apply<false>, grid, blk, 0, st, a, coef0, (long long)4 * C);
+    return check_launch("k_bn_bwd_finalize_apply");
+}
+
+extern "C" int gm_bn_bwd_finalize_apply_grouped_bf16(const gm_bn_bwd* ps, int G, float* stats, int rows, void* stream) {
+    return gm_bn_bwd_finalize_apply_grouped_bf16_ex(ps, G, stats, rows, 0, stream);
+}
diff --git a/greedy_multimodal_learning_amd/vtrunk.py b/greedy_multimodal_learning_amd/vtrunk.py
--- a/greedy_multimodal_learning_amd/vtrunk.py
+++ b/greedy_multimodal_learning_amd/vtrunk.py
@@ -24,6 +24,8 @@
 DS_DZ_LINK = True
 IDT_MASKED_ADDEND = True
 EPI_BN_BWD_STATS = True
+BN_FOLD = True
+DS_RES_AFFINE = True
 _GM_E_UNSUP = -3
 
 
@@ -338,8 +340,13 @@
                              dbs[g].data_ptr(), int(acc), 0, coef[g].data_ptr(), 0))
     st = L.stream_of(xb.device)
     arr = L.arr(L.BnBwd, descs)
-    L.check(lib.gm_bn_bwd_stats_finalize_grouped(arr, G, part.data_ptr(), rows, st), "gm_bn_bwd_stats_finalize_grouped")
-    L.check(lib.gm_bn_bwd_apply_grouped_bf16(arr, G, part.data_ptr(), rows, st), "gm_bn_bwd_apply_grouped_bf16")
+    if BN_FOLD:
+        L.check(lib.gm_bn_bwd_finalize_apply_grouped_bf16(arr, G, part.data_ptr(), rows, st),
+                "gm_bn_bwd_finalize_apply_grouped_bf16")
+    else:
+        L.check(lib.gm_bn_bwd_stats_finalize_grouped(arr, G, part.data_ptr(), rows, st),
+                "gm_bn_bwd_stats_finalize_grouped")
+        L.check(lib.gm_bn_bwd_apply_grouped_bf16(arr, G, part.data_ptr(), rows, st), "gm_bn_bwd_apply_grouped_bf16")
     if sunk:
         for p in list(gammas) + list(betas):
             sink_done(p)
@@ -381,10 +388,15 @@
         if stats is not None and "part" in stats:
             part, rows = stats.pop("part"), stats.pop("rows")
             st = L.stream_of(dev)
-            L.check(lib.gm_bn_fwd_stats_finalize_grouped(L.arr(L.BnFwd, descs), G, part.data_ptr(), rows, st),
-                    "gm_bn_fwd_stats_finalize_grouped")
-            L.check(lib.gm_bn_fwd_apply_grouped_bf16(L.arr(L.BnFwd, descs), G, part.data_ptr(), rows, st),
-                    "gm_bn_fwd_apply_grouped_bf16")
+            arr = L.arr(L.BnFwd, descs)
+            if BN_FOLD:
+                L.check(lib.gm_bn_fwd_finalize_apply_grouped_bf16(arr, G, part.data_ptr(), rows, st),
+                        "gm_bn_fwd_finalize_apply_grouped_bf16")
+            else:
+                L.check(lib.gm_bn_fwd_stats_finalize_grouped(arr, G, part.data_ptr(), rows, st),
+                        "gm_bn_fwd_stats_finalize_grouped")
+                L.check(lib.gm_bn_fwd_apply_grouped_bf16(arr, G, part.data_ptr(), rows, st),
+                        "gm_bn_fwd_apply_grouped_bf16")
         else:
             buf = _bn_scratch_g(dev, M, C, G)
             L.check(lib.gm_bn_fwd_train_grouped_bf16(L.arr(L.BnFwd, descs), G, buf.data_ptr(), buf.numel(),
@@ -454,6 +466,68 @@
     with torch.autocast("cuda", enabled=False):
         return _VBNFn.apply(X, residual, len(bns), bns, bool(relu), join, stats,
                             *[b.weight for b in bns], *[b.bias for b in bns])
+
+
+class _VBlockOutFn(torch.autograd.Function):
+
+    @staticmethod
+    def forward(ctx, Z, R, G, bns, rbns, st, rst, *params):
+        lib = L.load()
+        gammas, betas, rgammas, rbetas = (params[i * G:(i + 1) * G] for i in range(4))
+        zb, rb = _nhwc(Z.to(BF)), _nhwc(R.to(BF))
+        GN, C, H, W = zb.shape
+        N = GN // G
+        M = N * H * W
+        dev = zb.device
+        y = torch.empty_like(zb, memory_format=CL)
+        sm, si, smr, sir = (torch.empty(G, C, device=dev, dtype=torch.float32) for _ in range(4))
+        ymask = torch.empty(GN * H * W * C // 8, device=dev, dtype=torch.uint8)
+        descs, rdescs = [], []
+        for g in range(G):
+            r = slice(g * N, (g + 1) * N)
+            bn, rbn = bns[g], rbns[g]
+            descs.append(L.BnFwd(M, C, 1, zb[r].data_ptr(), rb[r].data_ptr(), y[r].data_ptr(),
+                                 gammas[g].data_ptr(), betas[g].data_ptr(), L.ptr(bn.running_mean),
+                                 L.ptr(bn.running_var), float(bn.momentum), float(bn.eps), sm[g].data_ptr(),
+                                 si[g].data_ptr(), L.ptr(bn.num_batches_tracked), 0,
+                                 ymask[g * (M * C // 8):].data_ptr()))
+            rdescs.append(L.BnFwd(M, C, 0, rb[r].data_ptr(), 0, 0, rgammas[g].data_ptr(), rbetas[g].data_ptr(),
+                                  L.ptr(rbn.running_mean), L.ptr(rbn.running_var), float(rbn.momentum),
+                                  float(rbn.eps), smr[g].data_ptr(), sir[g].data_ptr(),
+                                  L.ptr(rbn.num_batches_tracked), 0, 0))
+        part, rows = st.pop("part"), st.pop("rows")
+        rpart, rrows = rst.pop("part"), rst.pop("rows")
+        L.check(lib.gm_bn_fwd_finalize_apply_res_affine_grouped_bf16(
+            L.arr(L.BnFwd, descs), G, part.data_ptr(), rows, L.arr(L.BnFwd, rdescs), rpart.data_ptr(), rrows,
+            L.stream_of(dev)), "gm_bn_fwd_finalize_apply_res_affine_grouped_bf16")
+        ctx.save_for_backward(zb, rb, y, ymask, sm, si, smr, sir, *params)
+        ctx.G = G
+        return y
+
+    @staticmethod
+    def backward(ctx, dy):
+        zb, rb, y, ymask, sm, si, smr, sir, *prm = ctx.saved_tensors
+        G = ctx.G
+        gammas, betas, rgammas, rbetas = (prm[i * G:(i + 1) * G] for i in range(4))
+        need = ctx.needs_input_grad
+        want = [any(need[7 + i * G:7 + (i + 1) * G]) for i in range(4)]
+        dyb = _nhwc(dy.to(BF))
+        dz, _, gw, gb = _bn_backward(dyb, y, zb, G, gammas, betas, sm, si, True, False, None, want[0], want[1],
+                                     ymask)
+        dr, _, rgw, rgb = _bn_backward(dyb, y, rb, G, rgammas, rbetas, smr, sir, True, False, None, want[2],
+                                       want[3], ymask)
+        return (dz if need[0] else None, dr if need[1] else None, None, None, None, None, None,
+                *gw, *gb, *rgw, *rgb)
+
+
+def vblock_out(Z, R, bns, rbns, st, rst):
+    for group in (bns, rbns):
+        b0 = group[0]
+        if any(b.momentum is None or b.momentum != b0.momentum or b.eps != b0.eps for b in group):
+            raise L.GreedyMMLError("vtrunk BatchNorm: the views must share momentum and eps")
+    with torch.autocast("cuda", enabled=False):
+        return _VBlockOutFn.apply(Z, R, len(bns), bns, rbns, st, rst, *[b.weight for b in bns],
+                                  *[b.bias for b in bns], *[b.weight for b in rbns], *[b.bias for b in rbns])
 
 
 
@@ -668,19 +742,33 @@
         st = {"dgrad_link": link_in, "bn_link": link_out, "dz_link": res_link, "res_link": res_link}
         return vbn(vconv(x, convs, cjoin, stats=st), bns, stats=st, **kw)
     rl = {} if ds else None
-    if ds:
-        idt = cbn(X, [b.downsample[0] for b in blocks], [b.downsample[1] for b in blocks], join, res_link=rl)
+    dsbns = [b.downsample[1] for b in blocks] if ds else None
+    raw = None
+    if ds and DS_RES_AFFINE and DS_DZ_LINK and BN_RELU_MASK:
+        rst = {"dgrad_link": None, "bn_link": None, "dz_link": rl, "res_link": rl}
+        raw = (vconv(X, [b.downsample[0] for b in blocks], join, stats=rst), rst)
+        idt = None
+    elif ds:
+        idt = cbn(X, [b.downsample[0] for b in blocks], dsbns, join, res_link=rl)
     else:
         idt = X
+
+    def out_bn(x, convs, bns, link_in):
+        if raw is None:
+            return cbn(x, convs, bns, link_in=link_in, residual=idt, relu=True,
+                       residual_join=None if ds else join, res_link=rl)
+        st = {"dgrad_link": link_in, "bn_link": None, "dz_link": rl, "res_link": rl}
+        z = vconv(x, convs, None, stats=st)
+        if "part" in st and "part" in raw[1]:
+            return vblock_out(z, raw[0], bns, dsbns, st, raw[1])
+        return vbn(z, bns, stats=st, residual=vbn(raw[0], dsbns, stats=raw[1]), relu=True)
     l1 = {}
     out = cbn(X, [b.conv1 for b in blocks], [b.bn1 for b in blocks], join, link_out=l1, relu=True)
     if hasattr(b0, "conv3"):
         l2 = {}
         out = cbn(out, [b.conv2 for b in blocks], [b.bn2 for b in blocks], link_in=l1, link_out=l2, relu=True)
-        return cbn(out, [b.conv3 for b in blocks], [b.bn3 for b in blocks], link_in=l2, residual=idt, relu=True,
-                   residual_join=None if ds else join, res_link=rl)
-    return cbn(out, [b.conv2 for b in blocks], [b.bn2 for b in blocks], link_in=l1, residual=idt, relu=True,
-               residual_join=None if ds else join, res_link=rl)
+        return out_bn(out, [b.conv3 for b in blocks], [b.bn3 for b in blocks], l2)
+    return out_bn(out, [b.conv2 for b in blocks], [b.bn2 for b in blocks], l1)
 
 
 def vlayer(nets, i, X):
diff --git a/include/greedymml.h b/include/greedymml.h
--- a/include/greedymml.h
+++ b/include/greedymml.h
@@ -345,6 +345,18 @@
 size_t gm_bn_bwd_stats_coef_offset(int C, int G, int rows);
 int gm_bn_bwd_stats_finalize_grouped(const gm_bn_bwd* ps, int G, float* stats, int rows, void* stream);
 int gm_bn_bwd_apply_grouped_bf16(const gm_bn_bwd* ps, int G, const float* stats, int rows, void* stream);
+int gm_bn_fold_blocks(long long M, int C, int rows, int G);
+int gm_bn_fwd_finalize_apply_grouped_bf16(const gm_bn_fwd* ps, int G, float* stats, int rows, void* stream);
+int gm_bn_fwd_finalize_apply_grouped_bf16_ex(const gm_bn_fwd* ps, int G, float* stats, int rows, int nb,
+                                             void* stream);
+int gm_bn_bwd_finalize_apply_grouped_bf16(const gm_bn_bwd* ps, int G, float* stats, int rows, void* stream);
+int gm_bn_bwd_finalize_apply_grouped_bf16_ex(const gm_bn_bwd* ps, int G, float* stats, int rows, int nb,
+                                             void* stream);
+int gm_bn_fwd_finalize_apply_res_affine_grouped_bf16(const gm_bn_fwd* ps, int G, float* stats, int rows,
+                                                     const gm_bn_fwd* rps, float* rstats, int rrows, void* stream);
+int gm_bn_fwd_finalize_apply_res_affine_grouped_bf16_ex(const gm_bn_fwd* ps, int G, float* stats, int rows,
+                                                        const gm_bn_fwd* rps, float* rstats, int rrows, int nb,
+                                                        void* stream);
 int gm_bn_relu_maxpool2d_bwd_grouped_bf16(const gm_pool_desc* d, int G, const void* dy_pool, const void* idx,
                                           const void* xsel, const gm_bn_bwd* ps, void* scratch, size_t scratch_bytes,
                                           void* stream);
```

Result: faster. 37660 view-images/s, median of 6 (+2.4%).
